# bharatlytics/faceRecognition_InfrenceEngine

Measured on AMD Instinct MI355X. Metric: faces/sec end-to-end @1080p, higher is better.
Workload: dtype f16

## Files before the change

### facerecognition_infrenceengine_amd/_lib.py

```python
import ctypes as C
import struct
import os
import threading

_HERE = os.path.dirname(os.path.abspath(__file__))
LIB_PATH = os.path.join(_HERE, "csrc", "libfrhip.so")

_lock = threading.Lock()
_lib = None
ABI_VERSION = 106


class FrError(RuntimeError):
    pass


class ConvArgs(C.Structure):
    _fields_ = [("x", C.c_void_p), ("w", C.c_void_p), ("y", C.c_void_p),
                ("bias", C.c_void_p), ("slope", C.c_void_p), ("residual", C.c_void_p),
                ("out_f32_partial", C.c_void_p),
                ("B", C.c_int), ("H", C.c_int), ("W", C.c_int), ("Cin", C.c_int), ("Cout", C.c_int),
                ("KH", C.c_int), ("KW", C.c_int), ("stride", C.c_int), ("pad", C.c_int),
                ("Ho", C.c_int), ("Wo", C.c_int), ("bias_mode", C.c_int), ("splitk", C.c_int),
                ("x2", C.c_void_p), ("C2", C.c_int)]


class ConvStep(C.Structure):
    _fields_ = [("kind", C.c_int), ("args", ConvArgs)]


class ConvF8Args(C.Structure):
    _fields_ = [("x8", C.c_void_p), ("w8", C.c_void_p), ("y16", C.c_void_p), ("y8", C.c_void_p),
                ("oscale", C.c_void_p), ("bias", C.c_void_p), ("slope", C.c_void_p), ("residual", C.c_void_p),
                ("B", C.c_int), ("H", C.c_int), ("W", C.c_int), ("Cin", C.c_int), ("Cout", C.c_int),
                ("bias_mode", C.c_int), ("y8_mul", C.c_float), ("y8_sub", C.c_void_p)]


class RolePtr(C.c_void_p):
    role = None


class PnetLevel(C.Structure):
    _fields_ = [("x1", C.c_void_p), ("head", C.c_void_p), ("workspace", C.c_void_p), ("H1", C.c_int), ("W1", C.c_int),
                ("scale", C.c_float), ("boxes", C.c_void_p), ("scores", C.c_void_p), ("regs", C.c_void_p),
                ("counts", C.c_void_p), ("block_counts", C.c_void_p),
                ("x1s", C.c_void_p), ("hs", C.c_int), ("ws", C.c_int), ("f16", C.c_int)]


class FrameRef(C.Structure):
    _fields_ = [("data", C.c_void_p), ("H", C.c_int32), ("W", C.c_int32), ("nh", C.c_int32), ("nw", C.c_int32),
                ("reserved", C.c_int32 * 2)]


class Call(C.Structure):
    _fields_ = [("fn", C.c_int32), ("nargs", C.c_int32), ("a", C.c_uint64 * 22)]


_P, _I, _L, _F, _Z = C.c_void_p, C.c_int, C.c_int64, C.c_float, C.c_size_t
SEQ_FN = {"fr_dconv_mfma_f32": 1, "fr_pnet23_split_f16": 2, "fr_pnet_candidates": 3, "fr_sort_nms": 4, "fr_box_refine": 5,
          "fr_crop_conv1_f32": 6, "fr_stage_select": 7}

SIGNATURES = {
    "fr_version": (_I, []),
    "fr_last_error_string": (C.c_char_p, []),
    "fr_device_count": (_I, []),
    "fr_l2norm_rows_f32": (_I, [_P, _P, _I, _I, _P]),
    "fr_gallery_match_workspace": (_Z, [_I, _L]),
    "fr_gallery_match_f32": (_I, [_P, _P, _I, _L, _I, _L, _P, _P, _P, _Z, _P, _I, _P]),
    "fr_gallery_match_view_f32": (_I, [_P, _P, _P, _I, _L, _I, _P, _P, _P, _Z, _P]),
    "fr_gallery_topk_workspace": (_Z, [_I, _L, _I]),
    "fr_gallery_topk_f32": (_I, [_P, _P, _I, _L, _I, _I, _L, _P, _P, _P, _Z, _P, _I, _P]),
    "fr_gallery_topk_view_f32": (_I, [_P, _P, _P, _I, _L, _I, _I, _P, _P, _P, _Z, _P]),
    "fr_gallery_update_rows_f32": (_I, [_P, _P, _P, _I, _I, _I, _P]),
    "fr_gallery_match_f16_workspace": (_Z, [_I, _L]),
    "fr_gallery_match_f16": (_I, [_P, _P, _P, _I, _L, _I, _L, _P, _P, _P, _Z, _P, _I, _P]),
    "fr_gallery_match_f8_workspace": (_Z, [_I, _L]),
    "fr_gallery_match_f8": (_I, [_P, _P, _P, _I, _L, _I, _L, _P, _P, _P, _Z, _P, _I, _P]),
    "fr_gallery_update_rows_shadow": (_I, [_P, _P, _I, _P, _P, _I, _I, _I, _P]),
    "fr_gallery_match_view_f16_workspace": (_Z, [_I, _L]),
    "fr_gallery_match_view_f16": (_I, [_P, _P, _P, _P, _I, _L, _L, _I, _P, _P, _P, _Z, _P]),
    "fr_gallery_match_view_f8_workspace": (_Z, [_I, _L]),
    "fr_gallery_match_view_f8": (_I, [_P, _P, _P, _P, _I, _L, _L, _I, _P, _P, _P, _Z, _P]),
    "fr_gallery_topk_f16_workspace": (_Z, [_I, _L, _I]),
    "fr_gallery_topk_f16": (_I, [_P, _P, _P, _I, _L, _I, _I, _L, _P, _P, _P, _P, _P, _Z, _P, _I, _P]),
    "fr_gallery_topk_view_f16_workspace": (_Z, [_I, _L, _I]),
    "fr_gallery_topk_view_f16": (_I, [_P, _P, _P, _P, _I, _L, _L, _I, _I, _P, _P, _P, _P, _P, _Z, _P]),
    "fr_gallery_topk_view_masked_f32": (_I, [_P, _P, _P, _I, _L, _I, _I, _P, _P, _P, _Z, _P, _P]),
    "fr_gallery_match_grouped_workspace": (_Z, [_I, _L]),
    "fr_gallery_match_grouped_f32": (_I, [_P, _P, _P, _P, _P, _I, _I, _L, _L, _I, _P, _P, _P, _Z, _P, _I, _P]),
    "fr_gallery_topk_grouped_workspace": (_Z, [_I, _L, _I]),
    "fr_gallery_topk_grouped_f32": (_I, [_P, _P, _P, _P, _P, _I, _I, _L, _L, _I, _I, _P, _P, _P, _Z, _P, _I, _P]),
    "fr_gallery_gmax_update": (_I, [_P, _P, _L, _I, _P, _P]),
    "fr_f32_to_f8": (_I, [_P, _P, _L, _P]),
    "fr_f32_to_f16": (_I, [_P, _P, _L, _P]),
    "fr_match_decide": (_I, [_P, _P, _I, _F, _F, _P, _P]),
    "fr_match_pack_candidates": (_I, [_P, _P, _I, _P, _P]),
    "fr_match_reduce_shards": (_I, [_P, _I, _I, _I, _I, _P, _P, _P]),
    "fr_match_reduce_shards_topk": (_I, [_P, _I, _I, _I, _I, _I, _P, _P, _P]),
    "fr_exchange_pack_queries": (_I, [_P, _I, _I, _I, _P, _P]),
    "fr_exchange_counts": (_I, [_P, _I, _I, _I, _P, _P]),
    "fr_gallery_first_above_f32": (_I, [_P, _P, _I, _L, _I, _F, _I, _L, _P, _P, _P, _Z, _P]),
    "fr_cosine_matrix_f32": (_I, [_P, _P, _I, _I, _I, _P, _P]),
    "fr_mean_rows_f32": (_I, [_P, _I, _I, _P, _P]),
    "fr_unknown_assign_batch_f32": (_I, [_P, _P, _I, _I, _F, _P, _P, _P, _I, _I, _P, _P, _P, _P]),
    "fr_gallery_first_above_blocked_f32": (_I, [_P, _P, _P, _P, _I, _L, _I, _F, _I, _L, _P, _P, _P, _Z, _P]),
    "fr_enrol_batch_workspace": (_Z, [_I, _L]),
    "fr_enrol_batch_f32": (_I, [_P, _P, _I, _P, _P, _I, _P, _I, _I, _I, _P, _P, _L, _F, _F, _P, _P, _P, _P, _P, _P, _P, _P,
                                _Z, _P]),
    "fr_gallery_pairs_workspace": (_Z, [_L, _L]),
    "fr_gallery_pairs_above_f16": (_I, [_P, _P, _L, _I, _F, _I, _L, _I, _P, _P, _P, _P, _Z, _P]),
    "fr_conv_nhwc_f16": (_I, [C.POINTER(ConvArgs), _P]),
    "fr_conv_sequence": (_I, [C.POINTER(ConvStep), _I, _P]),
    "fr_conv_inblock_f16": (_I, [C.POINTER(ConvArgs), _P]),
    "fr_conv_nhwc_f8": (_I, [C.POINTER(ConvF8Args), _P]),
    "fr_quantize_f16_f8": (_I, [_P, _P, _L, _F, _P]),
    "fr_quantize_f16_f8_centred": (_I, [_P, _P, _L, _I, _P, _F, _P]),
    "fr_gptq_round_e4m3": (_I, [_P, _P, _P, _P, _I, _I, _P]),
    "fr_conv_stage14_weight_bytes": (_Z, [_I]),
    "fr_conv_stage14_pack": (_I, [_P, _P, _P]),
    "fr_conv_stage14_f16": (_I, [_P, _P, _P, _P, _I, _I, _P]),
    "fr_conv_walk64_weight_bytes": (_Z, [_I]),
    "fr_conv_walk64_pack": (_I, [_P, _P, _I, _P]),
    "fr_conv_walk64_f16": (_I, [_P, _P, _P, _P, _I, _P, _P, _I, _I, _I, _P]),
    "fr_conv_stage28_weight_bytes": (_Z, [_I]),
    "fr_conv_stage28_pack": (_I, [_P, _P, _P]),
    "fr_conv_stage28_f16": (_I, [_P, _P, _P, _P, _I, _I, _P]),
    "fr_conv_stage14_f8_weight_bytes": (_Z, [_I]),
    "fr_conv_stage14_f8_param_floats": (_Z, []),
    "fr_conv_stage14_f8_pack": (_I, [_P, _P, _P]),
    "fr_conv_stage14_f8": (_I, [_P, _P, _P, _P, _P, _I, _I, _P]),
    "fr_conv_splitk_epilogue": (_I, [_P, _I, _I, _I, _I, _I, _P, _I, _P, _P, _P, _P]),
    "fr_fc_reduce_l2norm": (_I, [_P, _I, _I, _I, _P, _P, _P, _P]),
    "fr_warp_affine_5pt": (_I, [_P, _I, _I, _I, _P, _P, _P, _I, _I, _P, _P, _P, _P]),
    "fr_warp_affine_5pt_slots": (_I, [_P, _I, _I, _I, _P, _P, _I, _I, _P, _P]),
    "fr_warp_affine_5pt_refs": (_I, [_P, _I, _P, _P, _P, _I, _I, _P, _P, _P, _P]),
    "fr_warp_affine_5pt_slots_refs": (_I, [_P, _I, _P, _P, _I, _I, _P, _P]),
    "fr_letterbox_u8": (_I, [_P, _I, _P, _I, _I, _P]),
    "fr_detections_unscale": (_I, [_P, _P, _P, _P, _I, _I, _P]),
    "fr_yuv420_to_bgr_u8": (_I, [_P, _P, _I, _I, _I, _I, _I, _I, _I, _I, _I, _I, _P]),
    "fr_yuv420_to_bgr_refs_u8": (_I, [_P, _P, _I, _I, _I, _I, _I, _I, _I, _I, _P]),
    "fr_frame_activity_u8": (_I, [_P, _I, _I, _I, _P, _I, _P, _P, _P, _I, _P, _P, _P, _I, _I, _I, _P]),
    "fr_frame_activity_refs_u8": (_I, [_P, _I, _P, _I, _P, _P, _P, _I, _P, _P, _P, _I, _I, _I, _P]),
    "fr_hud_draw_u8": (_I, [_P, _I, _I, _I, _P, _I, _P, _P, _I, _P, _I, _P]),
    "fr_hud_draw_refs_u8": (_I, [_P, _I, _P, _I, _P, _P, _I, _P, _I, _P]),
    "fr_track_associate_f32": (_I, [_P, _P, _P, _I, _I, _I, _I, _P, _P, _P, _F, _I, _I, _P, _P, _P, _P]),
    "fr_track_commit_f32": (_I, [_P, _P, _P, _P, _I, _I, _I, _I, _P, _P, _P, _P]),
    "fr_track_resolve_quality_i32": (_I, [_P, _P, _P, _P, _P, _P, _I, _I, _I, _I, _P, _P, _I, _P, _P, _P, _P]),
    "fr_track_fuse_f32": (_I, [_P, _P, _P, _P, _P, _P, _I, _I, _I, _I, _I, _F, _P, _P, _P, _P, _P, _P, _P]),
    "fr_face_quality_f16": (_I, [_P, _P, _P, _I, _I, _P, _P, _P, _F, _I, _I, _I, _I, _I, _F, _F, _F, _P]),
    "fr_pyramid_resize_norm":(_I, [_P, _I, _I, _I, _I, _I, _P, _P]),
    "fr_dconv_f32": (_I, [_P, _P, _P, _P, _P, _I, _I, _I, _I, _I, _I, _I, _I, _I, _P, _P, _I, _P]),
    "fr_dconv_mfma_f32": (_I, [_I, _P, _P, _P, _P, _P, _I, _I, _I, _P, _P, _P, _I, _I, _P, _I, _P, _P]),
    "fr_crop_conv1_f32": (_I, [_I, _P, _I, _I, _I, _P, _P, _I, _P, _P, _P, _P, _P]),
    "fr_crop_conv1_split": (_I, [_I, _P, _I, _I, _I, _P, _P, _I, _P, _P, _P, _P, _I, _P]),
    "fr_crop_conv1_list_f32": (_I, [_I, _P, _I, _I, _I, _P, _I, _P, _P, _I, _P, _P, _P, _P, _P]),
    "fr_ro_conv2_split": (_I, [_I, _P, _P, _P, _P, _P, _I, _P, _I, _P, _P]),
    "fr_ro_gemm_weight_bytes": (_Z, [_I]),
    "fr_ro_gemm_pack": (_I, [_I, _P, _P, _P]),
    "fr_ro_gemm_split": (_I, [_I, _P, _P, _P, _P, _P, _I, _P, _I, _P]),
    "fr_ro_margin_list": (_I, [_P, _I, _P, _I, _I, _F, _F, _P, _P, _I, _P]),
    "fr_ro_scatter_rows": (_I, [_P, _P, _P, _I, _I, _P, _P]),
    "fr_pnet23_workspace_bytes": (_Z, [_I, _I, _I]),
    "fr_pnet23_split_f16": (_I, [_P, _P, _I, _I, _I, _P, _P, _P, _P, _P, _P, _P, _P, _P, _I, _F, _F, _P, _P, _Z, _P]),
    "fr_maxpool_f32": (_I, [_P, _P, _I, _I, _I, _I, _I, _I, _P]),
    "fr_pnet_conv1_band": (_I, [_I, _P, _I, _I, _I, _I, _I, _P, _P, _P, _P, _P, _P, _P, _I, _P]),
    "fr_pnet_band_tiles_count": (_Z, [_I, _I, _I]),
    "fr_pnet_band_tiles": (_I, [_P, _I, _I, _I, _P, _P, _P]),
    "fr_pnet23_coarse_workspace_bytes": (_Z, [_I, _I, _I]),
    "fr_pnet23_coarse_f16": (_I, [_P, _P, _I, _I, _I, _P, _P, _P, _P, _P, _P, _P, _P, _P, _I, _F, _F, _P, _P, _Z, _F, _P, _Z, _P, _P]),
    "fr_pnet_pyramid_p23_coarse": (_I, [C.POINTER(PnetLevel), _I, _I, _P, _P, _P, _P, _P, _P, _P, _P, _I, _F, _F, _F, C.POINTER(_P), _P, _P]),
    "fr_pnet_finish_levels": (_I, [C.POINTER(PnetLevel), _I, _I, _P, _P, _P, _P, _P, _P, _P, _P, _F, _I, _F, _P, _P]),
    "fr_pnet_pyramid_conv1": (_I, [_I, _P, _I, _I, _I, C.POINTER(PnetLevel), _I, _P, _P, _P, _P, _P, _I, _P]),
    "fr_pnet_pyramid_p23": (_I, [C.POINTER(PnetLevel), _I, _I, _P, _P, _P, _P, _P, _P, _P, _P, _I, _F, _F, _P]),
    "fr_pnet_pyramid_band_tiles": (_I, [C.POINTER(PnetLevel), _I, _I, _P, _P, _P]),
    "fr_pnet_candidates": (_I, [_P, _I, _I, _I, _F, _F, _I, _P, _P, _P, _P, _P, _P, _P, _F, _P]),
    "fr_sort_nms": (_I, [_P, _P, _P, _I, _P, _I, _I, _I, _I, _F, _I, _I, _P, _P, _P, _P, _I, _P]),
    "fr_box_refine": (_I, [_P, _P, _I, _P, _I, _I, _I, _P]),
    "fr_crop_resize_norm": (_I, [_P, _I, _I, _I, _P, _P, _I, _I, _P, _P]),
    "fr_stage_select": (_I, [_P, _P, _I, _P, _I, _I, _F, _P, _P, _P, _I, _P, _P, _P]),
    "fr_detect_sequence": (_I, [C.POINTER(Call), _I]),
    "fr_det_conv_weight_halves": (_Z, [_I, _I, _I]),
    "fr_det_conv_f16": (_I, [_P, _P, _P, _P, _P, _I, _I, _I, _I, _I, _I, _I, _I, _I, _I, _I, _I, _I, _I, _I, _P]),
    "fr_det_conv_act_f16": (_I, [_P, _P, _P, _P, _P, _P, _I, _I, _I, _I, _I, _I, _I, _I, _I, _I, _I, _I, _I, _I, _I, _P]),
    "fr_dw_conv_f16": (_I, [_P, _P, _P, _P, _P, _I, _I, _I, _I, _I, _I, _I, _I, _I, _I, _P]),
    "fr_det_input_f16": (_I, [_P, _P, _I, _I, _I, _P]),
    "fr_det_pool_f16": (_I, [_P, _P, _I, _I, _I, _I, _I, _I, _I, _I, _I, _I, _P]),
    "fr_det_upsample_add_f16": (_I, [_P, _P, _P, _I, _I, _I, _I, _I, _P]),
    "fr_scrfd_decode": (_I, [_P, _P, _P, _I, _I, _I, _I, _I, _I, _F, _P, _I, _P, _P, _P, _P, _P]),
}

_NOCHECK = ("fr_version", "fr_device_count")


def _slot(v, t):
    if t is _F:
        return struct.unpack("<I", struct.pack("<f", float(v)))[0]
    if t is _P:
        if v is None:
            return 0
        return int(v.value or 0) if isinstance(v, C.c_void_p) else int(v)
    return int(v) & 0xFFFFFFFFFFFFFFFF


class Lib:

    def __init__(self, cdll):
        self._c = cdll
        self._calls = {}
        self._rec = threading.local()
        for name, (res, args) in SIGNATURES.items():
            fn = getattr(cdll, name)
            fn.restype = res
            fn.argtypes = args
            if res is _I and name not in _NOCHECK:
                self._calls[name] = self._checked(name, fn)
            else:
                self._calls[name] = fn

    def _checked(self, name, fn):
        err = self._c.fr_last_error_string

        fid, types, rec = SEQ_FN.get(name), fn.argtypes, self._rec

        def call(*a):
            rc = fn(*a)
            if rc != 0:
                raise FrError(f"{name} failed ({rc}): {err().decode()}")
            if getattr(rec, "calls", None) is not None:
                rec.invalid = name
            return rc

        def call_rec(*a):
            rc = fn(*a)
            if rc != 0:
                raise FrError(f"{name} failed ({rc}): {err().decode()}")
            calls = getattr(rec, "calls", None)
            if calls is not None:
                calls.append((fid, [_slot(v, t) for v, t in zip(a, types)],
                              [(i, v.role) for i, v in enumerate(a) if isinstance(v, RolePtr)]))
            return rc
        return call_rec if fid is not None else call

    def start_recording(self):
        self._rec.calls, self._rec.invalid = [], None

    def note(self, fid, *slots):
        calls = getattr(self._rec, "calls", None)
        if calls is not None:
            calls.append((fid, [int(v.value or 0) if isinstance(v, C.c_void_p) else int(v) for v in slots], []))

    def stop_recording(self):
        calls, self._rec.calls = getattr(self._rec, "calls", None), None
        self._rec.last_invalid = getattr(self._rec, "invalid", None)
        self._rec.invalid = None
        return None if self._rec.last_invalid else calls

    def recording_invalid(self):
        return getattr(self._rec, "last_invalid", None)

    def __getattr__(self, name):
        try:
            return self.__dict__["_calls"][name]
        except KeyError:
            raise AttributeError(name)


def load():
    global _lib
    with _lock:
        if _lib is None:
            import torch
            if not os.path.exists(LIB_PATH):
                raise FrError(f"{LIB_PATH} not built: run `python -c 'import __graft_entry__ as g; g.build()'` "
                              f"or `make -C {os.path.dirname(LIB_PATH)}`; there is no CPU fallback")
            lib = Lib(C.CDLL(LIB_PATH))
            have = lib.fr_version()
            if have != ABI_VERSION:
                raise FrError(f"{LIB_PATH} implements ABI version {have}, this binding needs {ABI_VERSION}: rebuild it "
                              f"(`make -C {os.path.dirname(LIB_PATH)}`)")
            _lib = lib
        return _lib


def ptr(t, role=None):
    if t is None:
        return None
    if role is None:
        return C.c_void_p(t.data_ptr())
    p = RolePtr(t.data_ptr())
    p.role = role
    return p


def stream_ptr():
    import torch
    return C.c_void_p(torch.cuda.current_stream().cuda_stream)


def require_gpu():
    import torch
    if not torch.cuda.is_available():
        raise FrError("no HIP device visible: this engine has no CPU path")
```

### facerecognition_infrenceengine_amd/csrc/pnet_fused.hip

```cpp
#include "detect_math.h"

#define P23_RH 8
#define P23_RW 32
#define P23_X1W (P23_RW + 4)
#define P23_X1PX ((P23_RH + 4) * P23_X1W)
#define P23_X2W (P23_RW + 2)
#define P23_X2PX ((P23_RH + 2) * P23_X2W)
#define P23_X2T ((P23_X2PX + 15) / 16)
#define P23_NT 512
#define P23_X1PL (448 * 32)
#define P23_X2PL (P23_X2PX * 32)

struct P23Args {
    const float* x1;
    const unsigned char* x1s;
    unsigned x1s_bytes;
    const float* w2; const float* b2; const float* s2;
    const float* w3; const float* b3; const float* s3;
    const float* hw; const float* hb;
    float* head;
    float* dl;
    int all_heads;
    int* list; int* counts; int seg_cap;
    float logit_thr;
    float band_hi;
    int B, H1, W1, H3, W3, tiles_x, tiles_y, ntiles;
    int* clist; int* ccounts;
    float coarse_thr;
    int* visited;
};

template <int NP, int NT>
__device__ __forceinline__ void p23_stage_weights(const P23Args& a, char* wf, float* cst) {
    const int tid = threadIdx.x;
    for (int e = tid; e < 15 * NP * 64; e += NT) {
        const int l2 = e & 63, plane = NP == 2 ? (e >> 6) & 1 : 0, slot = e / (64 * NP);
        const int r = l2 & 15, q = l2 >> 4;
        const bool c3 = slot >= 5;
        const int ct = c3 ? (slot - 5) / 5 : 0, ks = c3 ? (slot - 5) % 5 : slot;
        const float* w = (c3 ? a.w3 : a.w2) + ((size_t)(ct * 16 + r) * 10 + 2 * ks + (q >> 1)) * 16 + 8 * (q & 1);
        half8 o;
#pragma unroll
        for (int j = 0; j < 8; ++j) o[j] = split_f16_plane(w[j], plane);
        *reinterpret_cast<half8*>(wf + (size_t)e * 16) = o;
    }
    for (int e = tid; e < 16; e += NT) { cst[e] = a.b2[e]; cst[16 + e] = a.s2[e] - 1.f; }
    for (int e = tid; e < 32; e += NT) { cst[32 + e] = a.b3[e]; cst[64 + e] = a.s3[e] - 1.f; }
    for (int e = tid; e < 8; e += NT) cst[96 + e] = e < 6 ? a.hb[e] : 0.f;
}

template <bool COARSE>
__device__ __forceinline__ void pnet23_body(const P23Args& a, const int vb, const int vgrid, char* lds) {
#if defined(__HIP_DEVICE_COMPILE__)
    constexpr int NP = COARSE ? 1 : 2;
    char* x1t = lds;
    char* x2t = x1t + NP * P23_X1PL;
    char* wf = x2t + NP * P23_X2PL;
    float* cst = reinterpret_cast<float*>(wf + NP * 15 * 1024);
    int* lcnt = reinterpret_cast<int*>(cst + 104);
    const int tid = threadIdx.x, lane = tid & 63, wave = tid >> 6;
    const int fr = lane & 15, fq = lane >> 4;

    p23_stage_weights<NP, P23_NT>(a, wf, cst);
    if (tid == 0) *lcnt = 0;
    int* const seg = (COARSE ? a.clist : a.list) + (size_t)vb * a.seg_cap;

    int off2[5], off3[5];
#pragma unroll
    for (int ks = 0; ks < 5; ++ks) {
        int t = 2 * ks + (fq >> 1);
        if (t > 8) t = 8;
        off2[ks] = ((t / 3) * P23_X1W + t % 3) * 32 + (fq & 1) * 16;
        off3[ks] = ((t / 3) * P23_X2W + t % 3) * 32 + (fq & 1) * 16;
    }

    __amdgpu_buffer_rsrc_t xrs = buffer_rsrc(a.x1s, a.x1s_bytes);
    constexpr int NPIECE = 14 * NP, NI = (NPIECE + 7) / 8;
    int wy[NI], wx[NI], wc[NI];
#pragma unroll
    for (int i = 0; i < NI; ++i) {
        const int j = wave + 8 * i, pl = j >= 14 ? 1 : 0;
        const int p = (j - 14 * pl) * 32 + (lane >> 1);
        wy[i] = p < P23_X1PX ? p / P23_X1W : 1 << 20; wx[i] = p % P23_X1W;
        wc[i] = pl * 32 + (lane & 1) * 16;
    }
    auto issue_window = [&](int tile) {
        const int per = a.tiles_x * a.tiles_y;
        const int n = tile / per, rem = tile - n * per;
        const int ty0 = (rem / a.tiles_x) * P23_RH, tx0 = (rem % a.tiles_x) * P23_RW;
#pragma unroll
        for (int i = 0; i < NI; ++i) {
            const int j = wave + 8 * i;
            if (j < NPIECE) {
                const int gy = ty0 + wy[i], gx = tx0 + wx[i];
                const unsigned off = (gy < a.H1 && gx < a.W1) ? (unsigned)(((n * a.H1 + gy) * a.W1 + gx) * 64 + wc[i]) : 0x80000000u;
                __builtin_amdgcn_raw_ptr_buffer_load_lds(xrs, (lds_ptr_t)(x1t + (j >= 14 ? P23_X1PL + (j - 14) * 1024 : j * 1024)), 16, off, 0, 0, 0);
            }
        }
    };

    __syncthreads();
    half8 hwh, hwl;
#pragma unroll
    for (int j = 0; j < 8; ++j) {
        const int co = j < 4 ? 4 * fq + j : 16 + 4 * fq + (j - 4);
        const float w = fr < 6 ? a.hw[co * 6 + fr] : 0.f;
        split_f16(w, hwh, hwl, j);
    }
    (void)hwl;
    issue_window(vb);
    for (int tile = vb; tile < a.ntiles; tile += vgrid) {
        const int per = a.tiles_x * a.tiles_y;
        const int n = tile / per, rem = tile - n * per;
        const int ty0 = (rem / a.tiles_x) * P23_RH, tx0 = (rem % a.tiles_x) * P23_RW;
        asm volatile("s_waitcnt vmcnt(0)" ::: "memory");
        __syncthreads();
        {
            const int t0 = wave < 6 ? wave * 3 : 18 + (wave - 6) * 2, nt = wave < 6 ? 3 : 2;
            int pb[3];
            float4v acc[3];
#pragma unroll
            for (int t = 0; t < 3; ++t) {
                int q = (t0 + t) * 16 + fr;
                if (q >= P23_X2PX) q = 0;
                pb[t] = ((q / P23_X2W) * P23_X1W + q % P23_X2W) * 32;
                acc[t] = float4v{0.f, 0.f, 0.f, 0.f};
            }
#pragma unroll
            for (int ks = 0; ks < 5; ++ks) {
                const half8 ahi = *reinterpret_cast<const half8*>(wf + ((ks * NP + 0) * 64 + lane) * 16);
                if constexpr (COARSE) {
#pragma unroll
                    for (int t = 0; t < 3; ++t) {
                        if (t < nt) {
                            const half8 bhi = *reinterpret_cast<const half8*>(x1t + (pb[t] + off2[ks]));
                            acc[t] = __builtin_amdgcn_mfma_f32_16x16x32_f16(ahi, bhi, acc[t], 0, 0, 0);
                        }
                    }
                } else {
                    const half8 alo = *reinterpret_cast<const half8*>(wf + ((ks * 2 + 1) * 64 + lane) * 16);
#pragma unroll
                    for (int t = 0; t < 3; ++t) {
                        if (t < nt) {
                            const char* bp = x1t + (pb[t] + off2[ks]);
                            const half8 bhi = *reinterpret_cast<const half8*>(bp);
                            const half8 blo = *reinterpret_cast<const half8*>(bp + P23_X1PL);
                            acc[t] = __builtin_amdgcn_mfma_f32_16x16x32_f16(alo, bhi, acc[t], 0, 0, 0);
                            acc[t] = __builtin_amdgcn_mfma_f32_16x16x32_f16(ahi, blo, acc[t], 0, 0, 0);
                            acc[t] = __builtin_amdgcn_mfma_f32_16x16x32_f16(ahi, bhi, acc[t], 0, 0, 0);
                        }
                    }
                }
            }
            const float4v bb = *reinterpret_cast<const float4v*>(cst + 4 * fq), ss = *reinterpret_cast<const float4v*>(cst + 16 + 4 * fq);
#pragma unroll
            for (int t = 0; t < 3; ++t) {
                const int q = (t0 + t) * 16 + fr;
                if (t < nt && q < P23_X2PX) {
                    float4v v = acc[t] + bb;
#pragma unroll
                    for (int e = 0; e < 4; ++e) v[e] = __builtin_fmaf(fminf(v[e], 0.f), ss[e], v[e]);
                    char* o = x2t + q * 32 + fq * 8;
                    if constexpr (COARSE) {
                        half4 hi;
#pragma unroll
                        for (int e = 0; e < 4; ++e) hi[e] = (half_t)v[e];
                        *reinterpret_cast<half4*>(o) = hi;
                    } else {
                        half4 hi, lo;
#pragma unroll
                        for (int e = 0; e < 4; ++e) split_f16(v[e], hi, lo, e);
                        *reinterpret_cast<half4*>(o) = hi;
                        *reinterpret_cast<half4*>(o + P23_X2PL) = lo;
                    }
                }
            }
        }
        __syncthreads();
        if (tile + vgrid < a.ntiles) issue_window(tile + vgrid);
        {
            int pb[2];
            float4v acc[2][2];
#pragma unroll
            for (int t = 0; t < 2; ++t) {
                const int q = (wave * 2 + t) * 16 + fr;
                pb[t] = ((q >> 5) * P23_X2W + (q & 31)) * 32;
                acc[t][0] = acc[t][1] = float4v{0.f, 0.f, 0.f, 0.f};
            }
#pragma unroll
            for (int ks = 0; ks < 5; ++ks) {
                if constexpr (COARSE) {
                    half8 ahi[2];
#pragma unroll
                    for (int ct = 0; ct < 2; ++ct) ahi[ct] = *reinterpret_cast<const half8*>(wf + ((5 + ct * 5 + ks) * 64 + lane) * 16);
#pragma unroll
                    for (int t = 0; t < 2; ++t) {
                        const half8 bhi = *reinterpret_cast<const half8*>(x2t + (pb[t] + off3[ks]));
#pragma unroll
                        for (int ct = 0; ct < 2; ++ct) acc[t][ct] = __builtin_amdgcn_mfma_f32_16x16x32_f16(ahi[ct], bhi, acc[t][ct], 0, 0, 0);
                    }
                    continue;
                }
                half8 ahi[2], alo[2];
#pragma unroll
                for (int ct = 0; ct < 2; ++ct) {
                    ahi[ct] = *reinterpret_cast<const half8*>(wf + (((5 + ct * 5 + ks) * 2 + 0) * 64 + lane) * 16);
                    alo[ct] = *reinterpret_cast<const half8*>(wf + (((5 + ct * 5 + ks) * 2 + 1) * 64 + lane) * 16);
                }
#pragma unroll
                for (int t = 0; t < 2; ++t) {
                    const char* bp = x2t + (pb[t] + off3[ks]);
                    const half8 bhi = *reinterpret_cast<const half8*>(bp);
                    const half8 blo = *reinterpret_cast<const half8*>(bp + P23_X2PL);
#pragma unroll
                    for (int ct = 0; ct < 2; ++ct) {
                        acc[t][ct] = __builtin_amdgcn_mfma_f32_16x16x32_f16(alo[ct], bhi, acc[t][ct], 0, 0, 0);
                        acc[t][ct] = __builtin_amdgcn_mfma_f32_16x16x32_f16(ahi[ct], blo, acc[t][ct], 0, 0, 0);
                        acc[t][ct] = __builtin_amdgcn_mfma_f32_16x16x32_f16(ahi[ct], bhi, acc[t][ct], 0, 0, 0);
                    }
                }
            }
            const float4v b30 = *reinterpret_cast<const float4v*>(cst + 32 + 4 * fq), s30 = *reinterpret_cast<const float4v*>(cst + 64 + 4 * fq);
            const float4v b31 = *reinterpret_cast<const float4v*>(cst + 48 + 4 * fq), s31 = *reinterpret_cast<const float4v*>(cst + 80 + 4 * fq);
#pragma unroll
            for (int t = 0; t < 2; ++t) {
                float4v v0 = acc[t][0] + b30, v1 = acc[t][1] + b31;
                half8 bh, bl;
#pragma unroll
                for (int e = 0; e < 4; ++e) {
                    const float x0 = __builtin_fmaf(fminf(v0[e], 0.f), s30[e], v0[e]), x1 = __builtin_fmaf(fminf(v1[e], 0.f), s31[e], v1[e]);
                    const half_t h0 = (half_t)x0, h1 = (half_t)x1;
                    bh[e] = h0; bl[e] = (half_t)(x0 - (float)h0);
                    bh[4 + e] = h1; bl[4 + e] = (half_t)(x1 - (float)h1);
                }
                float4v d = {0.f, 0.f, 0.f, 0.f};
                if constexpr (!COARSE) {
                    d = __builtin_amdgcn_mfma_f32_16x16x32_f16(hwl, bh, d, 0, 0, 0);
                    d = __builtin_amdgcn_mfma_f32_16x16x32_f16(hwh, bl, d, 0, 0, 0);
                }
                d = __builtin_amdgcn_mfma_f32_16x16x32_f16(hwh, bh, d, 0, 0, 0);
                const int q = (wave * 2 + t) * 16 + fr;
                const int gy = ty0 + (q >> 5), gx = tx0 + (q & 31);
                const bool inb = fq < 2 && gy < a.H3 && gx < a.W3;
                const size_t cell = ((size_t)n * a.H3 + gy) * a.W3 + gx;
                const float4v hb4 = *reinterpret_cast<const float4v*>(cst + 96 + 4 * (fq & 1));
                const float o0 = d[0] + hb4[0], o1 = d[1] + hb4[1];
                const float dlv = __shfl(o1 - o0, fr, 64);
                const bool band = a.band_hi > a.logit_thr;
                const bool flag = inb && fq == 0 && (split_nonfinite(dlv) || (COARSE ? dlv >= a.coarse_thr : (dlv >= a.logit_thr && (!band || dlv <= a.band_hi))));
                const unsigned long long fm = __ballot(flag);
                if (fm) {
                    int base = 0;
                    if (lane == (int)__builtin_ctzll(fm)) base = atomicAdd(lcnt, (int)__builtin_popcountll(fm));
                    base = __shfl(base, (int)__builtin_ctzll(fm), 64);
                    if (flag) seg[base + (int)__builtin_popcountll(fm & ((1ull << lane) - 1ull))] = (int)cell;
                }
                if (inb) {
                    if (fq == 0) a.dl[cell] = o1 - o0;
                    if (!COARSE && (a.all_heads || (band && dlv >= a.logit_thr))) {
                        float* o = a.head + cell * 6 + 4 * fq;
                        *reinterpret_cast<float2*>(o) = make_float2(o0, o1);
                        if (fq == 0) *reinterpret_cast<float2*>(o + 2) = make_float2(d[2] + hb4[2], d[3] + hb4[3]);
                    }
                }
            }
        }
    }
    __syncthreads();
    if (tid == 0) (COARSE ? a.ccounts : a.counts)[vb] = *lcnt;
#endif
}

__global__ __launch_bounds__(P23_NT, 4) void pnet23_split_f16(P23Args a) {
    extern __shared__ __attribute__((aligned(16))) char lds[];
    pnet23_body<false>(a, (int)blockIdx.x, (int)gridDim.x, lds);
}
__global__ __launch_bounds__(P23_NT, 4) void pnet23_coarse_f16(P23Args a) {
    extern __shared__ __attribute__((aligned(16))) char lds[];
    pnet23_body<true>(a, (int)blockIdx.x, (int)gridDim.x, lds);
}

#define P23_MAXL 16
struct P23Levels {
    const unsigned char* x1s[P23_MAXL]; float* head[P23_MAXL]; float* dl[P23_MAXL];
    int H1[P23_MAXL], W1[P23_MAXL], seg_cap[P23_MAXL], first[P23_MAXL + 1];
    int nlevels;
};
__global__ __launch_bounds__(P23_NT, 4) void pnet23_split_levels(P23Args a, P23Levels t) {
    extern __shared__ __attribute__((aligned(16))) char lds[];
    int l = 0;
    while (l + 1 < t.nlevels && (int)blockIdx.x >= t.first[l + 1]) ++l;
    a.H1 = t.H1[l]; a.W1 = t.W1[l]; a.H3 = a.H1 - 4; a.W3 = a.W1 - 4;
    a.tiles_x = (a.W3 + P23_RW - 1) / P23_RW; a.tiles_y = (a.H3 + P23_RH - 1) / P23_RH;
    a.ntiles = a.B * a.tiles_x * a.tiles_y;
    a.x1s = t.x1s[l]; a.x1s_bytes = (unsigned)a.B * a.H1 * a.W1 * 64; a.head = t.head[l];
    a.dl = t.dl[l]; a.counts = reinterpret_cast<int*>(a.dl + (size_t)a.B * a.H3 * a.W3); a.list = a.counts + 512;
    a.seg_cap = t.seg_cap[l];
    pnet23_body<false>(a, (int)blockIdx.x - t.first[l], t.first[l + 1] - t.first[l], lds);
}

struct P23Coarse { int* buf[P23_MAXL]; };
__device__ __forceinline__ int p23_find_level(const P23Levels& t, const int g) {
    int l = 0;
    while (l + 1 < t.nlevels && g >= t.first[l + 1]) ++l;
    return l;
}
__device__ __forceinline__ void p23_set_level(P23Args& a, const P23Levels& t, const P23Coarse& c, const int l) {
    a.H1 = t.H1[l]; a.W1 = t.W1[l]; a.H3 = a.H1 - 4; a.W3 = a.W1 - 4;
    a.tiles_x = (a.W3 + P23_RW - 1) / P23_RW; a.tiles_y = (a.H3 + P23_RH - 1) / P23_RH;
    a.ntiles = a.B * a.tiles_x * a.tiles_y;
    a.x1s = t.x1s[l]; a.x1s_bytes = (unsigned)a.B * a.H1 * a.W1 * 64; a.head = t.head[l];
    a.dl = t.dl[l]; a.counts = reinterpret_cast<int*>(a.dl + (size_t)a.B * a.H3 * a.W3); a.list = a.counts + 512;
    a.seg_cap = t.seg_cap[l];
    a.ccounts = c.buf[l]; a.clist = c.buf[l] + 512;
}
__global__ __launch_bounds__(P23_NT, 4) void pnet23_coarse_levels(P23Args a, P23Levels t, P23Coarse c) {
    extern __shared__ __attribute__((aligned(16))) char lds[];
    const int l = p23_find_level(t, (int)blockIdx.x);
    p23_set_level(a, t, c, l);
    pnet23_body<true>(a, (int)blockIdx.x - t.first[l], t.first[l + 1] - t.first[l], lds);
}

#define P23R_NT 256
#define P23R_SLOT 1616
#define P23R_LO 800
#define P23R_LDS ((size_t)30 * 1024 + 108 * 4 + (P23R_NT / 64) * 16 * P23R_SLOT)
__global__ __launch_bounds__(P23R_NT, 1) void pnet23_reeval_levels(P23Args a, P23Levels t, P23Coarse c) {
#if defined(__HIP_DEVICE_COMPILE__)
    extern __shared__ __attribute__((aligned(16))) char lds[];
    char* wf = lds;
    float* cst = reinterpret_cast<float*>(wf + 30 * 1024);
    const int tid = threadIdx.x, lane = tid & 63, wave = tid >> 6;
    const int fr = lane & 15, fq = lane >> 4;
    char* const win = reinterpret_cast<char*>(cst + 108) + wave * (16 * P23R_SLOT);
    p23_stage_weights<2, P23R_NT>(a, wf, cst);
    half8 hwh, hwl;
#pragma unroll
    for (int j = 0; j < 8; ++j) {
        const int co = j < 4 ? 4 * fq + j : 16 + 4 * fq + (j - 4);
        const float w = fr < 6 ? a.hw[co * 6 + fr] : 0.f;
        split_f16(w, hwh, hwl, j);
    }
    __syncthreads();
    const float4v bb = *reinterpret_cast<const float4v*>(cst + 4 * fq), ss = *reinterpret_cast<const float4v*>(cst + 16 + 4 * fq);
    const float4v b30 = *reinterpret_cast<const float4v*>(cst + 32 + 4 * fq), s30 = *reinterpret_cast<const float4v*>(cst + 64 + 4 * fq);
    const float4v b31 = *reinterpret_cast<const float4v*>(cst + 48 + 4 * fq), s31 = *reinterpret_cast<const float4v*>(cst + 80 + 4 * fq);
    const float4v hb4 = *reinterpret_cast<const float4v*>(cst + 96 + 4 * (fq & 1));
    const bool band = a.band_hi > a.logit_thr;
    char* const xc = win + fr * P23R_SLOT + (fq & 1) * 16;
    int pj[25], psrc[25], pdst[25];
    const int nseg = t.first[t.nlevels];
    for (int g = (int)blockIdx.x * (P23R_NT / 64) + wave; g < nseg; g += (int)gridDim.x * (P23R_NT / 64)) {
        const int l = p23_find_level(t, g);
        p23_set_level(a, t, c, l);
        const int vb = g - t.first[l];
        const int n_list = a.ccounts[vb];
        const int* const lst = a.clist + (size_t)vb * a.seg_cap;
        int* const seg = a.list + (size_t)vb * a.seg_cap;
        const int hw3 = a.H3 * a.W3;
        int nflag = 0;
        if (a.visited && lane == 0 && n_list) atomicAdd(a.visited, n_list);
#pragma unroll
        for (int it = 0; it < 25; ++it) {
            const int idx = it * 64 + lane, j = idx / 100, rem = idx - j * 100, px = rem >> 2, ch = rem & 3;
            pj[it] = j;
            psrc[it] = ((px / 5) * a.W1 + px % 5) * 64 + ch * 16;
            pdst[it] = j * P23R_SLOT + (ch >> 1) * P23R_LO + px * 32 + (ch & 1) * 16;
        }
        auto corner_of = [&](int i0) {
            const int cell = lst[min(i0 + fr, n_list - 1)];
            const int n = cell / hw3, rem = cell - n * hw3, y = rem / a.W3, x = rem - y * a.W3;
            return ((n * a.H1 + y) * a.W1 + x) * 64;
        };
        float4v pf[25];
        if (n_list > 0) {
            const int corner = corner_of(0);
#pragma unroll
            for (int it = 0; it < 25; ++it)
                pf[it] = *reinterpret_cast<const float4v*>(a.x1s + (size_t)(unsigned)(__shfl(corner, pj[it], 64) + psrc[it]));
        }
        for (int i0 = 0; i0 < n_list; i0 += 16) {
            const int cell = lst[min(i0 + fr, n_list - 1)];
#pragma unroll
            for (int it = 0; it < 25; ++it) *reinterpret_cast<float4v*>(win + pdst[it]) = pf[it];
            __builtin_amdgcn_wave_barrier();
            if (i0 + 16 < n_list) {
                const int corner = corner_of(i0 + 16);
#pragma unroll
                for (int it = 0; it < 25; ++it)
                    pf[it] = *reinterpret_cast<const float4v*>(a.x1s + (size_t)(unsigned)(__shfl(corner, pj[it], 64) + psrc[it]));
            }
            float4v acc2[9];
#pragma unroll
            for (int p = 0; p < 9; ++p) acc2[p] = float4v{0.f, 0.f, 0.f, 0.f};
#pragma unroll
            for (int ks = 0; ks < 5; ++ks) {
                int tp = 2 * ks + (fq >> 1);
                if (tp > 8) tp = 8;
                const half8 ahi = *reinterpret_cast<const half8*>(wf + ((ks * 2 + 0) * 64 + lane) * 16);
                const half8 alo = *reinterpret_cast<const half8*>(wf + ((ks * 2 + 1) * 64 + lane) * 16);
#pragma unroll
                for (int p = 0; p < 9; ++p) {
                    const char* bp = xc + ((p / 3 + tp / 3) * 5 + (p % 3 + tp % 3)) * 32;
                    const half8 bhi = *reinterpret_cast<const half8*>(bp);
                    const half8 blo = *reinterpret_cast<const half8*>(bp + P23R_LO);
                    acc2[p] = __builtin_amdgcn_mfma_f32_16x16x32_f16(alo, bhi, acc2[p], 0, 0, 0);
                    acc2[p] = __builtin_amdgcn_mfma_f32_16x16x32_f16(ahi, blo, acc2[p], 0, 0, 0);
                    acc2[p] = __builtin_amdgcn_mfma_f32_16x16x32_f16(ahi, bhi, acc2[p], 0, 0, 0);
                }
            }
            __builtin_amdgcn_wave_barrier();
#pragma unroll
            for (int p = 0; p < 9; ++p) {
                float4v v = acc2[p] + bb;
#pragma unroll
                for (int e = 0; e < 4; ++e) v[e] = __builtin_fmaf(fminf(v[e], 0.f), ss[e], v[e]);
                half4 hi, lo;
#pragma unroll
                for (int e = 0; e < 4; ++e) split_f16(v[e], hi, lo, e);
                char* o = win + fr * P23R_SLOT + p * 32 + fq * 8;
                *reinterpret_cast<half4*>(o) = hi;
                *reinterpret_cast<half4*>(o + P23R_LO) = lo;
            }
            __builtin_amdgcn_wave_barrier();
            float4v acc3[2] = {float4v{0.f, 0.f, 0.f, 0.f}, float4v{0.f, 0.f, 0.f, 0.f}};
#pragma unroll
            for (int ks = 0; ks < 5; ++ks) {
                int tp = 2 * ks + (fq >> 1);
                if (tp > 8) tp = 8;
                const half8 bhi = *reinterpret_cast<const half8*>(xc + tp * 32);
                const half8 blo = *reinterpret_cast<const half8*>(xc + tp * 32 + P23R_LO);
#pragma unroll
                for (int ct = 0; ct < 2; ++ct) {
                    const half8 ahi = *reinterpret_cast<const half8*>(wf + (((5 + ct * 5 + ks) * 2 + 0) * 64 + lane) * 16);
                    const half8 alo = *reinterpret_cast<const half8*>(wf + (((5 + ct * 5 + ks) * 2 + 1) * 64 + lane) * 16);
                    acc3[ct] = __builtin_amdgcn_mfma_f32_16x16x32_f16(alo, bhi, acc3[ct], 0, 0, 0);
                    acc3[ct] = __builtin_amdgcn_mfma_f32_16x16x32_f16(ahi, blo, acc3[ct], 0, 0, 0);
                    acc3[ct] = __builtin_amdgcn_mfma_f32_16x16x32_f16(ahi, bhi, acc3[ct], 0, 0, 0);
                }
            }
            __builtin_amdgcn_wave_barrier();
            const float4v v0 = acc3[0] + b30, v1 = acc3[1] + b31;
            half8 bh, bl;
#pragma unroll
            for (int e = 0; e < 4; ++e) {
                const float x0 = __builtin_fmaf(fminf(v0[e], 0.f), s30[e], v0[e]), x1 = __builtin_fmaf(fminf(v1[e], 0.f), s31[e], v1[e]);
                const half_t h0 = (half_t)x0, h1 = (half_t)x1;
                bh[e] = h0; bl[e] = (half_t)(x0 - (float)h0);
                bh[4 + e] = h1; bl[4 + e] = (half_t)(x1 - (float)h1);
            }
            float4v d = {0.f, 0.f, 0.f, 0.f};
            d = __builtin_amdgcn_mfma_f32_16x16x32_f16(hwl, bh, d, 0, 0, 0);
            d = __builtin_amdgcn_mfma_f32_16x16x32_f16(hwh, bl, d, 0, 0, 0);
            d = __builtin_amdgcn_mfma_f32_16x16x32_f16(hwh, bh, d, 0, 0, 0);
            const bool inb = fq < 2 && i0 + fr < n_list;
            const float o0 = d[0] + hb4[0], o1 = d[1] + hb4[1];
            const float dlv = __shfl(o1 - o0, fr, 64);
            const bool flag = inb && fq == 0 && (split_nonfinite(dlv) || (dlv >= a.logit_thr && (!band || dlv <= a.band_hi)));
            const unsigned long long fm = __ballot(flag);
            if (flag) seg[nflag + (int)__builtin_popcountll(fm & ((1ull << lane) - 1ull))] = cell;
            nflag += (int)__builtin_popcountll(fm);
            if (inb) {
                if (fq == 0) a.dl[cell] = o1 - o0;
                if (band && dlv >= a.logit_thr) {
                    float* o = a.head + (size_t)cell * 6 + 4 * fq;
                    *reinterpret_cast<float2*>(o) = make_float2(o0, o1);
                    if (fq == 0) *reinterpret_cast<float2*>(o + 2) = make_float2(d[2] + hb4[2], d[3] + hb4[3]);
                }
            }
        }
        if (lane == 0) a.counts[vb] = nflag;
    }
#endif
}

#define PREF_WS 304
struct PRefArgs {
    const float* x1; const float* w2; const float* b2; const float* s2; const float* w3; const float* b3; const float* s3;
    const float* hw; const float* hb; float* head;
    const int* list; const int* counts; int seg_cap;
    int B, H1, W1, H3, W3;
    int* counter;
};

__device__ __forceinline__ void pnet_refine_body(const PRefArgs& a, const int block, float (*wins)[16 * PREF_WS], int (*cbase)[16]) {
#if defined(__HIP_DEVICE_COMPILE__)
    const int tid = threadIdx.x, lane = tid & 63, wave = tid >> 6;
    const int li = lane & 15, kq = lane >> 4;
    float* win = wins[wave];
    if (a.counts[block] <= wave * 16) return;
    float wa2[27], wa3[2][36], hwa[8];
#pragma unroll
    for (int s = 0; s < 27; ++s) wa2[s] = a.w2[(li * 10 + s / 3) * 16 + 4 * (s % 3) + kq];
#pragma unroll
    for (int i = 0; i < 2; ++i)
#pragma unroll
        for (int s = 0; s < 36; ++s) wa3[i][s] = a.w3[((16 * i + li) * 10 + s / 4) * 16 + 4 * (s % 4) + kq];
#pragma unroll
    for (int i = 0; i < 2; ++i)
#pragma unroll
        for (int e = 0; e < 4; ++e) hwa[i * 4 + e] = li < 6 ? a.hw[(16 * i + 4 * kq + e) * 6 + li] : 0.f;
    const float4v b2 = *reinterpret_cast<const float4v*>(a.b2 + 4 * kq), s2 = *reinterpret_cast<const float4v*>(a.s2 + 4 * kq);
    float4v b3[2], s3[2], hb4;
#pragma unroll
    for (int i = 0; i < 2; ++i) {
        b3[i] = *reinterpret_cast<const float4v*>(a.b3 + 16 * i + 4 * kq);
        s3[i] = *reinterpret_cast<const float4v*>(a.s3 + 16 * i + 4 * kq);
    }
#pragma unroll
    for (int r = 0; r < 4; ++r) hb4[r] = kq * 4 + r < 6 ? a.hb[kq * 4 + r] : 0.f;

    const int hw3 = a.H3 * a.W3;
    {
        const int* lst = a.list + (size_t)block * a.seg_cap;
        const int n_list = a.counts[block];
        if (a.counter && tid == 0 && n_list) atomicAdd(a.counter, n_list);
        for (int i0 = wave * 16; i0 < n_list; i0 += 64) {
            {
                const int c = lst[min(i0 + li, n_list - 1)];
                const int n = c / hw3, r = c - n * hw3, y = r / a.W3, x = r - y * a.W3;
                if (kq == 0) cbase[wave][li] = ((n * a.H1 + y) * a.W1 + x) * 12;
            }
            __builtin_amdgcn_wave_barrier();
            int l_ = lane;
            asm volatile("" : "+v"(l_));
            float4v pf[19];
#pragma unroll
            for (int it = 0; it < 19; ++it) {
                const int idx = min(it * 64 + l_, 1199);
                const int j = idx / 75, rem = idx - j * 75, row = rem / 15, c4 = rem - row * 15;
                pf[it] = *reinterpret_cast<const float4v*>(a.x1 + (size_t)(unsigned)cbase[wave][j] + (row * a.W1 * 12 + c4 * 4));
            }
#pragma unroll
            for (int it = 0; it < 19; ++it) {
                const int idx = it * 64 + l_;
                const int j = idx / 75, rem = idx - j * 75, row = rem / 15, c4 = rem - row * 15;
                if (it < 18 || l_ < 48) *reinterpret_cast<float4v*>(win + j * PREF_WS + row * 60 + c4 * 4) = pf[it];
            }
            __builtin_amdgcn_wave_barrier();
            const float* xb = win + li * PREF_WS + kq;
            float4v acc2[9];
#pragma unroll
            for (int p = 0; p < 9; ++p) acc2[p] = float4v{0.f, 0.f, 0.f, 0.f};
#pragma unroll
            for (int s = 0; s < 27; ++s) {
                const int tap = s / 3, c4 = s - tap * 3, ty = tap / 3, tx = tap - ty * 3;
#pragma unroll
                for (int p = 0; p < 9; ++p) {
                    const int py = p / 3, px = p - py * 3;
                    acc2[p] = __builtin_amdgcn_mfma_f32_16x16x4f32(wa2[s], xb[((py + ty) * 5 + px + tx) * 12 + 4 * c4], acc2[p], 0, 0, 0);
                }
            }
            __builtin_amdgcn_wave_barrier();
#pragma unroll
            for (int p = 0; p < 9; ++p) {
                float4v v = acc2[p] + b2;
#pragma unroll
                for (int e = 0; e < 4; ++e) v[e] = v[e] > 0.f ? v[e] : v[e] * s2[e];
                *reinterpret_cast<float4v*>(win + li * PREF_WS + p * 16 + 4 * kq) = v;
            }
            __builtin_amdgcn_wave_barrier();
            float4v acc3[2] = {float4v{0.f, 0.f, 0.f, 0.f}, float4v{0.f, 0.f, 0.f, 0.f}};
#pragma unroll
            for (int s = 0; s < 36; ++s) {
                const float bv = xb[(s / 4) * 16 + 4 * (s % 4)];
#pragma unroll
                for (int i = 0; i < 2; ++i) acc3[i] = __builtin_amdgcn_mfma_f32_16x16x4f32(wa3[i][s], bv, acc3[i], 0, 0, 0);
            }
            float4v hd = hb4;
#pragma unroll
            for (int i = 0; i < 2; ++i) {
                float4v v = acc3[i] + b3[i];
#pragma unroll
                for (int e = 0; e < 4; ++e) v[e] = v[e] > 0.f ? v[e] : v[e] * s3[i][e];
#pragma unroll
                for (int e = 0; e < 4; ++e) hd = __builtin_amdgcn_mfma_f32_16x16x4f32(hwa[i * 4 + e], v[e], hd, 0, 0, 0);
            }
            if (i0 + li < n_list && kq < 2) {
                float* o = a.head + (size_t)lst[i0 + li] * 6 + 4 * kq;
                *reinterpret_cast<float2*>(o) = make_float2(hd[0], hd[1]);
                if (kq == 0) *reinterpret_cast<float2*>(o + 2) = make_float2(hd[2], hd[3]);
            }
            __builtin_amdgcn_wave_barrier();
        }
    }
#endif
}

__global__ __launch_bounds__(256, 2) void pnet_refine_mfma(PRefArgs a) {
    __shared__ __attribute__((aligned(16))) float wins[4][16 * PREF_WS];
    __shared__ int cbase[4][16];
    pnet_refine_body(a, blockIdx.x, wins, cbase);
}

#define PREF_MAXL 16
struct PRefLevels {
    const float* x1[PREF_MAXL]; float* head[PREF_MAXL]; const int* list[PREF_MAXL]; const int* counts[PREF_MAXL];
    int seg_cap[PREF_MAXL], H1[PREF_MAXL], W1[PREF_MAXL], first[PREF_MAXL + 1];
    int nlevels;
};
__global__ __launch_bounds__(256, 2) void pnet_refine_levels(PRefArgs a, PRefLevels t) {
    __shared__ __attribute__((aligned(16))) float wins[4][16 * PREF_WS];
    __shared__ int cbase[4][16];
    int l = 0;
    while (l + 1 < t.nlevels && (int)blockIdx.x >= t.first[l + 1]) ++l;
    a.x1 = t.x1[l]; a.head = t.head[l]; a.list = t.list[l]; a.counts = t.counts[l]; a.seg_cap = t.seg_cap[l];
    a.H1 = t.H1[l]; a.W1 = t.W1[l]; a.H3 = t.H1[l] - 4; a.W3 = t.W1[l] - 4;
    pnet_refine_body(a, (int)blockIdx.x - t.first[l], wins, cbase);
}

static void p23_layout(int B, int H1, int W1, long long& ncell, long long& ntiles, int& grid, int& seg_cap) {
    const int H3 = H1 - 4, W3 = W1 - 4;
    ncell = (long long)B * H3 * W3;
    ntiles = (long long)B * ((W3 + P23_RW - 1) / P23_RW) * ((H3 + P23_RH - 1) / P23_RH);
    grid = (int)(ntiles < 512 ? ntiles : 512);
    seg_cap = (int)((ntiles + grid - 1) / (grid > 0 ? grid : 1)) * (P23_RH * P23_RW);
}
extern "C" size_t fr_pnet23_workspace_bytes(int B, int H1, int W1) {
    if (B <= 0 || H1 < 5 || W1 < 5) return 0;
    long long ncell, ntiles; int grid, seg_cap;
    p23_layout(B, H1, W1, ncell, ntiles, grid, seg_cap);
    return (size_t)ncell * 4 + 512 * 4 + (size_t)grid * seg_cap * 4;
}

extern "C" size_t fr_pnet23_coarse_workspace_bytes(int B, int H1, int W1) {
    if (B <= 0 || H1 < 5 || W1 < 5) return 0;
    long long ncell, ntiles; int grid, seg_cap;
    p23_layout(B, H1, W1, ncell, ntiles, grid, seg_cap);
    return 512 * 4 + (size_t)grid * seg_cap * 4;
}

static unsigned p23_reeval_grid(long long segments) {
    const long long blocks = (segments + P23R_NT / 64 - 1) / (P23R_NT / 64);
    return (unsigned)(blocks < 256 ? blocks : 256);
}

constexpr size_t P23_LDS = (size_t)2 * P23_X1PL + (size_t)2 * P23_X2PL + 30 * 1024 + 108 * 4;
constexpr size_t P23C_LDS = (size_t)P23_X1PL + (size_t)P23_X2PL + 15 * 1024 + 108 * 4;

static int p23_level(const char* who, const float* x1, const void* x1s, int B, int H1, int W1, const float* w2, const float* b2,
                     const float* s2, const float* w3, const float* b3, const float* s3, const float* hw,
                     const float* hb, float* head, int all_heads, float refine_logit_thr, float refine_band_hi,
                     int32_t* refined_count, void* workspace, size_t workspace_bytes, float coarse_margin, void* coarse,
                     size_t coarse_bytes, int32_t* visited_count, fr_stream_t stream);

extern "C" int fr_pnet23_split_f16(const float* x1, const void* x1s, int B, int H1, int W1, const float* w2, const float* b2,
                                   const float* s2, const float* w3, const float* b3, const float* s3, const float* hw,
                                   const float* hb, float* head, int all_heads, float refine_logit_thr, float refine_band_hi,
                                   int32_t* refined_count, void* workspace, size_t workspace_bytes, fr_stream_t stream) {
    return p23_level("fr_pnet23_split_f16", x1, x1s, B, H1, W1, w2, b2, s2, w3, b3, s3, hw, hb, head, all_heads, refine_logit_thr,
                     refine_band_hi, refined_count, workspace, workspace_bytes, 0.f, nullptr, 0, nullptr, stream);
}

extern "C" int fr_pnet23_coarse_f16(const float* x1, const void* x1s, int B, int H1, int W1, const float* w2, const float* b2,
                                    const float* s2, const float* w3, const float* b3, const float* s3, const float* hw,
                                    const float* hb, float* head, int all_heads, float refine_logit_thr, float refine_band_hi,
                                    int32_t* refined_count, void* workspace, size_t workspace_bytes, float coarse_margin,
                                    void* coarse, size_t coarse_bytes, int32_t* visited_count, fr_stream_t stream) {
    FR_REQUIRE(!(all_heads & 1), "fr_pnet23_coarse_f16: all_heads & 1 (the approximate heads of every cell) needs fr_pnet23_split_f16");
    FR_REQUIRE(coarse && coarse_margin >= 0.f, "fr_pnet23_coarse_f16: needs a coarse buffer and a margin >= 0");
    return p23_level("fr_pnet23_coarse_f16", x1, x1s, B, H1, W1, w2, b2, s2, w3, b3, s3, hw, hb, head, all_heads, refine_logit_thr,
                     refine_band_hi, refined_count, workspace, workspace_bytes, coarse_margin, coarse, coarse_bytes, visited_count, stream);
}

static int p23_level(const char* who, const float* x1, const void* x1s, int B, int H1, int W1, const float* w2, const float* b2,
                     const float* s2, const float* w3, const float* b3, const float* s3, const float* hw,
                     const float* hb, float* head, int all_heads, float refine_logit_thr, float refine_band_hi,
                     int32_t* refined_count, void* workspace, size_t workspace_bytes, float coarse_margin, void* coarse,
                     size_t coarse_bytes, int32_t* visited_count, fr_stream_t stream) {
    FR_REQUIRE(x1 && x1s && w2 && b2 && s2 && w3 && b3 && s3 && hw && hb && head, "%s: null pointer", who);
    FR_REQUIRE((int64_t)B * H1 * W1 * 64 < (1ll << 31), "%s: the split conv1 map must stay below 2 GiB (got %lld bytes)", who, (long long)B * H1 * W1 * 64);
    FR_REQUIRE(B > 0 && H1 >= 5 && W1 >= 5, "%s: the conv1 map must be at least 5x5 (got %dx%d)", who, H1, W1);
    P23Args a;
    a.x1 = x1; a.x1s = (const unsigned char*)x1s; a.x1s_bytes = (unsigned)((int64_t)B * H1 * W1 * 64); a.w2 = w2; a.b2 = b2; a.s2 = s2; a.w3 = w3; a.b3 = b3; a.s3 = s3; a.hw = hw; a.hb = hb; a.head = head; a.all_heads = all_heads & 1;
    a.B = B; a.H1 = H1; a.W1 = W1; a.H3 = H1 - 4; a.W3 = W1 - 4;
    a.tiles_x = (a.W3 + P23_RW - 1) / P23_RW; a.tiles_y = (a.H3 + P23_RH - 1) / P23_RH;
    long long ncell, nt; int grid, seg_cap;
    p23_layout(B, H1, W1, ncell, nt, grid, seg_cap);
    FR_REQUIRE(nt < (1ll << 31) && ncell < (1ll << 31), "%s: too many tiles", who);
    const size_t need = fr_pnet23_workspace_bytes(B, H1, W1);
    FR_REQUIRE(workspace && workspace_bytes >= need, "%s: workspace needs %zu bytes (fr_pnet23_workspace_bytes)", who, need);
    a.dl = reinterpret_cast<float*>(workspace);
    a.counts = reinterpret_cast<int*>(a.dl + ncell);
    a.list = a.counts + 512;
    a.seg_cap = seg_cap;
    a.logit_thr = refine_logit_thr;
    a.band_hi = refine_band_hi;
    a.ntiles = (int)nt;
    a.clist = a.ccounts = a.visited = nullptr; a.coarse_thr = 0.f;
    hipStream_t s = fr_stream(stream);
    if (coarse) {
        const size_t cneed = fr_pnet23_coarse_workspace_bytes(B, H1, W1);
        FR_REQUIRE(coarse_bytes >= cneed, "%s: the coarse buffer needs %zu bytes (fr_pnet23_coarse_workspace_bytes)", who, cneed);
        a.ccounts = reinterpret_cast<int*>(coarse); a.clist = a.ccounts + 512;
        a.coarse_thr = refine_logit_thr - coarse_margin; a.visited = visited_count;
        static FrDevLatch latch0, latch1;
        if (!fr_raise_lds(reinterpret_cast<const void*>(pnet23_coarse_f16), P23C_LDS, latch0) ||
            !fr_raise_lds(reinterpret_cast<const void*>(pnet23_reeval_levels), P23R_LDS, latch1)) { fr_set_error("fr_pnet23_coarse_f16: cannot raise dynamic LDS"); return FR_E_LAUNCH; }
        pnet23_coarse_f16<<<grid, P23_NT, P23C_LDS, s>>>(a);
        FR_CHECK_LAUNCH("pnet23_coarse_f16");
        P23Levels t{};
        P23Coarse c{};
        t.nlevels = 1; t.x1s[0] = a.x1s; t.head[0] = head; t.dl[0] = a.dl; t.H1[0] = H1; t.W1[0] = W1; t.seg_cap[0] = seg_cap;
        t.first[0] = 0; t.first[1] = grid; c.buf[0] = a.ccounts;
        pnet23_reeval_levels<<<p23_reeval_grid(grid), P23R_NT, P23R_LDS, s>>>(a, t, c);
        FR_CHECK_LAUNCH("pnet23_reeval_levels");
    } else {
        static FrDevLatch latch;
        if (!fr_raise_lds(reinterpret_cast<const void*>(pnet23_split_f16), P23_LDS, latch)) { fr_set_error("fr_pnet23_split_f16: cannot raise dynamic LDS"); return FR_E_LAUNCH; }
        pnet23_split_f16<<<grid, P23_NT, P23_LDS, s>>>(a);
        FR_CHECK_LAUNCH("pnet23_split_f16");
    }
    if (all_heads & 2) return FR_OK;
    PRefArgs r;
    r.x1 = x1; r.w2 = w2; r.b2 = b2; r.s2 = s2; r.w3 = w3; r.b3 = b3; r.s3 = s3; r.hw = hw; r.hb = hb; r.head = head;
    r.list = a.list; r.counts = a.counts; r.seg_cap = seg_cap;
    r.B = B; r.H1 = H1; r.W1 = W1; r.H3 = a.H3; r.W3 = a.W3; r.counter = refined_count;
    pnet_refine_mfma<<<grid, 256, 0, s>>>(r);
    FR_CHECK_LAUNCH("pnet_refine_mfma");
    return FR_OK;
}

int fr_pnet_candidates_levels_launch(const fr_pnet_level* lv, int nlevels, int nframes, float thr, int cap, float dl_min, hipStream_t s);

extern "C" int fr_pnet_finish_levels(const fr_pnet_level* levels, int nlevels, int nframes, const float* w2, const float* b2,
                                     const float* s2, const float* w3, const float* b3, const float* s3, const float* hw,
                                     const float* hb, float thr, int cap, float dl_min, int32_t* refined_count, fr_stream_t stream) {
    FR_REQUIRE(levels && nlevels > 0 && nlevels <= PREF_MAXL && nframes > 0 && cap > 0, "fr_pnet_finish_levels: 1 .. %d levels", PREF_MAXL);
    FR_REQUIRE(w2 && b2 && s2 && w3 && b3 && s3 && hw && hb, "fr_pnet_finish_levels: null pointer");
    PRefLevels t;
    t.nlevels = nlevels;
    int total = 0;
    for (int l = 0; l < nlevels; ++l) {
        const fr_pnet_level& L = levels[l];
        FR_REQUIRE(L.x1 && L.head && L.workspace && L.boxes && L.scores && L.regs && L.counts && L.block_counts && L.H1 >= 5 && L.W1 >= 5 && L.scale > 0.f,
                   "fr_pnet_finish_levels: level %d: bad entry", l);
        long long ncell, nt; int grid, seg_cap;
        p23_layout(nframes, L.H1, L.W1, ncell, nt, grid, seg_cap);
        float* dl = reinterpret_cast<float*>(L.workspace);
        const int* counts = reinterpret_cast<const int*>(dl + ncell);
        t.x1[l] = L.x1; t.head[l] = L.head; t.counts[l] = counts; t.list[l] = counts + 512;
        t.seg_cap[l] = seg_cap; t.H1[l] = L.H1; t.W1[l] = L.W1;
        t.first[l] = total;
        total += grid;
    }
    t.first[nlevels] = total;
    PRefArgs r;
    r.x1 = nullptr; r.w2 = w2; r.b2 = b2; r.s2 = s2; r.w3 = w3; r.b3 = b3; r.s3 = s3; r.hw = hw; r.hb = hb; r.head = nullptr;
    r.list = nullptr; r.counts = nullptr; r.seg_cap = 0; r.B = nframes; r.H1 = r.W1 = r.H3 = r.W3 = 0; r.counter = refined_count;
    hipStream_t s = fr_stream(stream);
    pnet_refine_levels<<<total, 256, 0, s>>>(r, t);
    FR_CHECK_LAUNCH("pnet_refine_levels");
    return fr_pnet_candidates_levels_launch(levels, nlevels, nframes, thr, cap, dl_min, s);
}

__global__ __launch_bounds__(256) void pnet_band_tiles_kernel(const int* __restrict__ list, const int* __restrict__ counts, int seg_cap,
                                                             int H3, int W3, int regions_x, int regions_y, int32_t* __restrict__ tbuf,
                                                             int32_t* __restrict__ tiles) {
    const int n_list = counts[blockIdx.x];
    const int* lst = list + (size_t)blockIdx.x * seg_cap;
    const int hw3 = H3 * W3;
    for (int i = threadIdx.x; i < n_list; i += 256) {
        const int c = lst[i];
        const int n = c / hw3, r = c - n * hw3, y = r / W3, x = r - y * W3;
        const int ry0 = (2 * y) >> 4, ry1 = min((2 * y + 9) >> 4, regions_y - 1);
        const int rx0 = (2 * x) >> 6, rx1 = min((2 * x + 9) >> 6, regions_x - 1);
        for (int ry = ry0; ry <= ry1; ++ry)
            for (int rx = rx0; rx <= rx1; ++rx) {
                const int t = (n * regions_y + ry) * regions_x + rx;
                const unsigned bit = 1u << (t & 31);
                const unsigned old = atomicOr(reinterpret_cast<unsigned*>(tbuf) + 1 + (t >> 5), bit);
                if (!(old & bit)) tiles[atomicAdd(tbuf, 1)] = t;
            }
    }
}

extern "C" size_t fr_pnet_band_tiles_count(int B, int H1, int W1) {
    if (B <= 0 || H1 < 5 || W1 < 5) return 0;
    return (size_t)B * ((H1 + 7) / 8) * ((W1 + 31) / 32);
}

extern "C" int fr_pnet_band_tiles(const void* workspace, int B, int H1, int W1, int32_t* tbuf, int32_t* tiles, fr_stream_t stream) {
    FR_REQUIRE(workspace && tbuf && tiles && B > 0 && H1 >= 5 && W1 >= 5, "fr_pnet_band_tiles: bad argument");
    long long ncell, nt; int grid, seg_cap;
    p23_layout(B, H1, W1, ncell, nt, grid, seg_cap);
    const float* dl = reinterpret_cast<const float*>(workspace);
    const int* counts = reinterpret_cast<const int*>(dl + ncell);
    const int regions_y = (H1 + 7) / 8, regions_x = (W1 + 31) / 32;
    const size_t ntile = (size_t)B * regions_y * regions_x;
    hipStream_t s = fr_stream(stream);
    if (hipMemsetAsync(tbuf, 0, (1 + (ntile + 31) / 32) * sizeof(int32_t), s) != hipSuccess) { fr_set_error("fr_pnet_band_tiles: memset failed"); return FR_E_LAUNCH; }
    pnet_band_tiles_kernel<<<grid, 256, 0, s>>>(counts + 512, counts, seg_cap, H1 - 4, W1 - 4, regions_x, regions_y, tbuf, tiles);
    FR_CHECK_LAUNCH("pnet_band_tiles_kernel");
    return FR_OK;
}

static int p23_pyramid(const char* who, const fr_pnet_level* levels, int nlevels, int nframes, const float* w2, const float* b2,
                       const float* s2, const float* w3, const float* b3, const float* s3, const float* hw,
                       const float* hb, int all_heads, float refine_logit_thr, float refine_band_hi, float coarse_margin,
                       void* const* coarse, int32_t* visited_count, fr_stream_t stream);

extern "C" int fr_pnet_pyramid_p23(const fr_pnet_level* levels, int nlevels, int nframes, const float* w2, const float* b2,
                                   const float* s2, const float* w3, const float* b3, const float* s3, const float* hw,
                                   const float* hb, int all_heads, float refine_logit_thr, float refine_band_hi, fr_stream_t stream) {
    return p23_pyramid("fr_pnet_pyramid_p23", levels, nlevels, nframes, w2, b2, s2, w3, b3, s3, hw, hb, all_heads, refine_logit_thr,
                       refine_band_hi, 0.f, nullptr, nullptr, stream);
}

extern "C" int fr_pnet_pyramid_p23_coarse(const fr_pnet_level* levels, int nlevels, int nframes, const float* w2, const float* b2,
                                          const float* s2, const float* w3, const float* b3, const float* s3, const float* hw,
                                          const float* hb, int all_heads, float refine_logit_thr, float refine_band_hi,
                                          float coarse_margin, void* const* coarse, int32_t* visited_count, fr_stream_t stream) {
    FR_REQUIRE(!(all_heads & 1), "fr_pnet_pyramid_p23_coarse: all_heads & 1 (the approximate heads of every cell) needs fr_pnet_pyramid_p23");
    FR_REQUIRE(coarse && coarse_margin >= 0.f, "fr_pnet_pyramid_p23_coarse: needs the coarse buffers and a margin >= 0");
    return p23_pyramid("fr_pnet_pyramid_p23_coarse", levels, nlevels, nframes, w2, b2, s2, w3, b3, s3, hw, hb, all_heads, refine_logit_thr,
                       refine_band_hi, coarse_margin, coarse, visited_count, stream);
}

static int p23_pyramid(const char* who, const fr_pnet_level* levels, int nlevels, int nframes, const float* w2, const float* b2,
                       const float* s2, const float* w3, const float* b3, const float* s3, const float* hw,
                       const float* hb, int all_heads, float refine_logit_thr, float refine_band_hi, float coarse_margin,
                       void* const* coarse, int32_t* visited_count, fr_stream_t stream) {
    FR_REQUIRE(levels && nlevels > 0 && nlevels <= P23_MAXL && nframes > 0, "%s: 1 .. %d levels", who, P23_MAXL);
    FR_REQUIRE(w2 && b2 && s2 && w3 && b3 && s3 && hw && hb, "%s: null pointer", who);
    P23Levels t;
    P23Coarse c{};
    t.nlevels = nlevels;
    long long total = 0;
    for (int l = 0; l < nlevels; ++l) {
        const fr_pnet_level& L = levels[l];
        if (coarse) {
            FR_REQUIRE(coarse[l], "%s: level %d: no coarse buffer", who, l);
            c.buf[l] = reinterpret_cast<int*>(coarse[l]);
        }
        FR_REQUIRE(L.x1s && L.head && L.workspace && L.H1 >= 5 && L.W1 >= 5, "%s: level %d: bad entry", who, l);
        FR_REQUIRE((int64_t)nframes * L.H1 * L.W1 * 64 < (1ll << 31), "%s: level %d: the split conv1 map must stay below 2 GiB", who, l);
        long long ncell, nt; int grid, seg_cap;
        p23_layout(nframes, L.H1, L.W1, ncell, nt, grid, seg_cap);
        t.x1s[l] = reinterpret_cast<const unsigned char*>(L.x1s); t.head[l] = L.head; t.dl[l] = reinterpret_cast<float*>(L.workspace);
        t.H1[l] = L.H1; t.W1[l] = L.W1; t.seg_cap[l] = seg_cap;
        t.first[l] = (int)total;
        total += grid;
    }
    t.first[nlevels] = (int)total;
    P23Args a{};
    a.w2 = w2; a.b2 = b2; a.s2 = s2; a.w3 = w3; a.b3 = b3; a.s3 = s3; a.hw = hw; a.hb = hb; a.all_heads = all_heads & 1;
    a.logit_thr = refine_logit_thr; a.band_hi = refine_band_hi; a.B = nframes;
    if (coarse) {
        a.coarse_thr = refine_logit_thr - coarse_margin; a.visited = visited_count;
        static FrDevLatch latch0, latch1;
        if (!fr_raise_lds(reinterpret_cast<const void*>(pnet23_coarse_levels), P23C_LDS, latch0) ||
            !fr_raise_lds(reinterpret_cast<const void*>(pnet23_reeval_levels), P23R_LDS, latch1)) { fr_set_error("fr_pnet_pyramid_p23_coarse: cannot raise dynamic LDS"); return FR_E_LAUNCH; }
        pnet23_coarse_levels<<<(unsigned)total, P23_NT, P23C_LDS, fr_stream(stream)>>>(a, t, c);
        FR_CHECK_LAUNCH("pnet23_coarse_levels");
        pnet23_reeval_levels<<<p23_reeval_grid(total), P23R_NT, P23R_LDS, fr_stream(stream)>>>(a, t, c);
        FR_CHECK_LAUNCH("pnet23_reeval_levels");
        return FR_OK;
    }
    static FrDevLatch latch;
    if (!fr_raise_lds(reinterpret_cast<const void*>(pnet23_split_levels), P23_LDS, latch)) { fr_set_error("fr_pnet_pyramid_p23: cannot raise dynamic LDS"); return FR_E_LAUNCH; }
    pnet23_split_levels<<<(unsigned)total, P23_NT, P23_LDS, fr_stream(stream)>>>(a, t);
    FR_CHECK_LAUNCH("pnet23_split_levels");
    return FR_OK;
}

struct PBandLevels {
    const int* counts[PREF_MAXL];
    int seg_cap[PREF_MAXL], H1[PREF_MAXL], W1[PREF_MAXL], word0[PREF_MAXL], level[PREF_MAXL], first[PREF_MAXL + 1];
    int nlevels;
};
__global__ __launch_bounds__(256) void pnet_band_tiles_levels(PBandLevels t, int32_t* __restrict__ tbuf, int32_t* __restrict__ tiles, int cap) {
    int l = 0;
    while (l + 1 < t.nlevels && (int)blockIdx.x >= t.first[l + 1]) ++l;
    const int b = (int)blockIdx.x - t.first[l];
    const int n_list = t.counts[l][b];
    const int* lst = t.counts[l] + 512 + (size_t)b * t.seg_cap[l];
    const int H3 = t.H1[l] - 4, W3 = t.W1[l] - 4, hw3 = H3 * W3;
    const int regions_y = (t.H1[l] + 7) / 8, regions_x = (t.W1[l] + 31) / 32;
    unsigned* bitmap = reinterpret_cast<unsigned*>(tbuf) + 1 + t.word0[l];
    for (int i = threadIdx.x; i < n_list; i += 256) {
        const int c = lst[i];
        const int n = c / hw3, r = c - n * hw3, y = r / W3, x = r - y * W3;
        const int ry0 = (2 * y) >> 4, ry1 = min((2 * y + 9) >> 4, regions_y - 1);
        const int rx0 = (2 * x) >> 6, rx1 = min((2 * x + 9) >> 6, regions_x - 1);
        for (int ry = ry0; ry <= ry1; ++ry)
            for (int rx = rx0; rx <= rx1; ++rx) {
                const int tl = (n * regions_y + ry) * regions_x + rx;
                const unsigned bit = 1u << (tl & 31);
                const unsigned old = atomicOr(bitmap + (tl >> 5), bit);
                if (!(old & bit)) {
                    const int at = atomicAdd(tbuf, 1);
                    if (at < cap) tiles[at] = (t.level[l] << 27) | tl;
                }
            }
    }
}

extern "C" int fr_pnet_pyramid_band_tiles(const fr_pnet_level* levels, int nlevels, int nframes, int32_t* tbuf, int32_t* tiles,
                                          fr_stream_t stream) {
    FR_REQUIRE(levels && nlevels > 0 && nlevels <= PREF_MAXL && nframes > 0 && tbuf && tiles, "fr_pnet_pyramid_band_tiles: bad argument");
    PBandLevels t;
    t.nlevels = 0;
    long long blocks = 0, words = 0, cap = 0;
    for (int l = 0; l < nlevels; ++l) {
        const fr_pnet_level& L = levels[l];
        if (!L.f16) continue;
        FR_REQUIRE(L.workspace && L.H1 >= 5 && L.W1 >= 5, "fr_pnet_pyramid_band_tiles: level %d: bad entry", l);
        long long ncell, nt; int grid, seg_cap;
        p23_layout(nframes, L.H1, L.W1, ncell, nt, grid, seg_cap);
        const long long ntile = (long long)fr_pnet_band_tiles_count(nframes, L.H1, L.W1);
        FR_REQUIRE(ntile < (1ll << 27), "fr_pnet_pyramid_band_tiles: level %d: too many tiles", l);
        const int k = t.nlevels++;
        t.counts[k] = reinterpret_cast<const int*>(reinterpret_cast<const float*>(L.workspace) + ncell);
        t.seg_cap[k] = seg_cap; t.H1[k] = L.H1; t.W1[k] = L.W1; t.word0[k] = (int)words; t.level[k] = l;
        t.first[k] = (int)blocks;
        blocks += grid; words += (ntile + 31) / 32; cap += ntile;
    }
    FR_REQUIRE(t.nlevels > 0 && cap < (1ll << 31), "fr_pnet_pyramid_band_tiles: no level in the f16 form");
    t.first[t.nlevels] = (int)blocks;
    hipStream_t s = fr_stream(stream);
    if (hipMemsetAsync(tbuf, 0, (size_t)(1 + words) * sizeof(int32_t), s) != hipSuccess) { fr_set_error("fr_pnet_pyramid_band_tiles: memset failed"); return FR_E_LAUNCH; }
    pnet_band_tiles_levels<<<(unsigned)blocks, 256, 0, s>>>(t, tbuf, tiles, (int)cap);
    FR_CHECK_LAUNCH("pnet_band_tiles_levels");
    return FR_OK;
}
```

### facerecognition_infrenceengine_amd/mtcnn.py

```python
import contextlib
import ctypes
import functools
import logging
import math
import threading
from types import SimpleNamespace
from typing import NamedTuple

import torch

from . import _lib


def pyramid_scales(h, w, minsize=20, factor=0.709):
    m = 12.0 / minsize
    minl = min(h, w) * m
    scales, k = [], 0
    while minl >= 12:
        scales.append(m * factor ** k)
        minl *= factor
        k += 1
    return scales


def _pool_out(n, k, s):
    o = -(-(n - k) // s) + 1
    if (o - 1) * s >= n:
        o -= 1
    return o


MFMA_LAYERS = {0: (3, 12, 3, 3, 1), 1: (12, 16, 3, 3, 1), 2: (16, 32, 3, 3, 2),
               10: (4, 28, 3, 3, 2), 11: (28, 48, 3, 3, 3), 12: (48, 64, 2, 2, 4), 13: (64, 128, 3, 3, 4),
               14: (128, 6, 1, 1, 1),
               20: (4, 32, 3, 3, 1), 21: (32, 64, 3, 3, 2), 22: (64, 64, 3, 3, 4), 23: (64, 128, 2, 2, 4),
               24: (128, 256, 3, 3, 4), 25: (256, 16, 1, 1, 1)}


class _MConv:

    def __init__(self, layer, w, b, slope, device, head=None):
        cin, cout, kh, kw, ntb = MFMA_LAYERS[layer]
        rcout, rcin = w.shape[0], w.shape[1]
        assert tuple(w.shape[2:]) == (kh, kw) and rcout <= cout and rcin <= cin, (layer, tuple(w.shape))
        wfull = torch.zeros((cout, cin, kh, kw), dtype=torch.float32)
        wfull[:rcout, :rcin] = w
        w = wfull
        bfull = torch.zeros(cout); bfull[:rcout] = b; b = bfull
        if slope is not None:
            sfull = torch.zeros(cout); sfull[:rcout] = slope; slope = sfull
        self.layer, self.cin, self.cout, self.kh, self.kw = layer, cin, cout, kh, kw
        cinp = -(-cin // 4) * 4
        cp = ntb * 16 + (16 if ntb % 2 == 0 else 0)
        gsz = ntb * 16
        ngroups = -(-cout // gsz)
        wp = torch.zeros((ngroups, kh * kw, cinp, cp), dtype=torch.float32)
        wt = w.permute(2, 3, 1, 0).reshape(kh * kw, cin, cout)
        for g in range(ngroups):
            n = min(gsz, cout - g * gsz)
            wp[g, :, :cin, :n] = wt[:, :, g * gsz:g * gsz + n]
        self.w = wp.contiguous().to(device)
        bp = torch.zeros(ngroups * gsz); bp[:cout] = b
        self.b = bp.to(device)
        self.slope = None
        if slope is not None:
            sp = torch.zeros(ngroups * gsz); sp[:cout] = slope
            self.slope = sp.to(device)
        self.head_w = self.head_b = None
        self.nhead = 0
        if head is not None:
            self.head_w = head[0].t().contiguous().to(torch.float32).to(device)
            self.head_b = head[1].to(torch.float32).contiguous().to(device)
            self.nhead = head[0].shape[0]
        self.pool = {0: 2, 10: 3, 11: 3, 20: 3, 21: 3, 22: 2}.get(layer, 0)

    def out_hw(self, h, w):
        hc, wc = h - self.kh + 1, w - self.kw + 1
        return (_pool_out(hc, self.pool, 2), _pool_out(wc, self.pool, 2)) if self.pool else (hc, wc)


_CHAINS = {"pnet": (("conv1", ("conv2",)), ("conv2", ("conv3",)), ("conv3", ("conv4_1", "conv4_2"))),
           "rnet": (("conv1", ("conv2",)), ("conv2", ("conv3",)), ("conv3", ("dense4",)), ("dense4", ("dense5_1", "dense5_2"))),
           "onet": (("conv1", ("conv2",)), ("conv2", ("conv3",)), ("conv3", ("conv4",)), ("conv4", ("dense5",)),
                    ("dense5", ("dense6_1", "dense6_2", "dense6_3")))}


def canonical_scale(state, net, dead_zone=2):
    st = dict(state)
    for name, readers in _CHAINS[net]:
        w = st[name + ".weight"]
        rms = float(w.double().pow(2).mean().sqrt())
        if rms == 0.0:
            continue
        e = math.log2(math.sqrt(2.0 / w[0].numel()) / rms)
        k = int(round(e)) if abs(e) > dead_zone else 0
        if k:
            st[name + ".weight"] = w * 2.0 ** k
            st[name + ".bias"] = st[name + ".bias"] * 2.0 ** k
            for n in readers:
                st[n + ".weight"] = st[n + ".weight"] * 2.0 ** -k
    return st


def _dense_as_conv(w, k, c):
    o = w.shape[0]
    return w.reshape(o, k, k, c).permute(0, 3, 2, 1).contiguous()


class DetectSettings:
    SINGLE_FRAME_LEVEL_STREAMS = 4
    one_stream = False
    level_streams = 2
    phase_marks = None
    solo_max_frames = 7
    pnet_band = True
    split_pconv1 = True
    split_pconv1_min_px = 10000
    pyramid_launch = True
    refined_cells = None
    use_sequence = True
    fused_crop = True
    split_ro = True
    coarse_p23 = True
    coarse_margin = 0.05
    visited_cells = None

    def __init__(self, minsize=20, factor=0.709, fused_pnet=True, batch_min_pixels=None):
        self.minsize, self.factor = minsize, factor
        self.fused_pnet = bool(fused_pnet)
        self.batch_min_pixels = 22_000_000 if batch_min_pixels is None else int(batch_min_pixels)
        self.single_frame_level_streams = self.SINGLE_FRAME_LEVEL_STREAMS


class DetectPlan(NamedTuple):
    N: int
    scales: tuple
    geo: tuple
    batch: bool
    few: bool
    band: bool
    fused: tuple
    f16: tuple
    pyramid: bool
    solo: bool
    nside: int
    cache: bool
    recorder: bool
    split: bool
    coarse: float
    chunks: tuple


def _is_batch(cfg, N, H, W):
    return N * H * W >= cfg.batch_min_pixels


def _level_geo(H, W, scale):
    hs, ws = int(math.ceil(H * scale)), int(math.ceil(W * scale))
    return hs, ws, _pool_out(hs - 2, 2, 2), _pool_out(ws - 2, 2, 2)


def _frames32(h, w):
    return (2 ** 31 - 1) // (h * w * 64)


def _f16_conv1(cfg, band, h, w):
    return bool(band and cfg.split_pconv1 and h * w >= cfg.split_pconv1_min_px)


def detect_plan(N, H, W, cfg, trace=False, level_streams=None, out=False, capturing=False):
    return _plan(N, H, W, tuple([getattr(cfg, k) for k in _PLAN_READS]), cfg.phase_marks is None and cfg.refined_cells is None,
                 trace, level_streams, out, capturing)


_PLAN_READS = ("minsize", "factor", "fused_pnet", "batch_min_pixels", "solo_max_frames", "pnet_band", "split_pconv1", "split_pconv1_min_px",
               "pyramid_launch", "one_stream", "level_streams", "single_frame_level_streams", "split_ro", "fused_crop", "use_sequence",
               "coarse_p23", "coarse_margin")


@functools.lru_cache(maxsize=256)
def _plan(N, H, W, settings, recordable, trace, level_streams, out, capturing):
    cfg = SimpleNamespace(**dict(zip(_PLAN_READS, settings)))
    scales = tuple(pyramid_scales(H, W, cfg.minsize, cfg.factor))
    geo = tuple(_level_geo(H, W, s) for s in scales)
    batch = _is_batch(cfg, N, H, W)
    few = N <= cfg.solo_max_frames and not batch
    fusable = bool(cfg.fused_pnet) and not trace
    chunks, per = (), N
    if fusable and not out and N > 1 and geo and 1 <= _frames32(*geo[0][2:]) < N:
        per = -(-N // -(-N // _frames32(*geo[0][2:])))
        chunks = tuple((n0, min(N, n0 + per)) for n0 in range(0, N, per))
    band = bool(cfg.pnet_band and batch and not trace)
    fused = tuple(bool(cfg.fused_pnet) and per <= _frames32(h, w) for _, _, h, w in geo)
    f16 = tuple(fu and _f16_conv1(cfg, band, h, w) for fu, (_, _, h, w) in zip(fused, geo))
    pyramid = bool(cfg.pyramid_launch and batch and fusable and all(fused))
    nside = max(1, min(2, level_streams if level_streams is not None else cfg.level_streams))
    own = few and level_streams is None
    if own and capturing and cfg.single_frame_level_streams > 0:
        nside = min(cfg.single_frame_level_streams, max(1, len(scales) - 1))
    eager = bool(trace or cfg.one_stream or (own and not capturing))
    cache = bool(eager and few and not trace and not out and not capturing)
    recorder = bool(cache and recordable and cfg.use_sequence and cfg.fused_pnet and cfg.fused_crop and not cfg.one_stream)
    split = bool(cfg.split_ro and cfg.fused_crop and batch and not trace)
    coarse = float(cfg.coarse_margin) if cfg.coarse_p23 and band else 0.0
    return DetectPlan(N, scales, geo, batch, few, band, fused, f16, pyramid, eager or pyramid, nside, cache, recorder, split, coarse, chunks)


_RO = (SimpleNamespace(name="rnet", cap_in="cap_p", cap_out="cap_r", crop=24, map1=(11, 28), map2=(4, 48), w1="_rc1", w2="_rc2",
                       layers=("r1", "r2", "r3", "r4", "r5"), nhead=6, naux=4, refine=1),
       SimpleNamespace(name="onet", cap_in="cap_r", cap_out="cap_o", crop=48, map1=(23, 32), map2=(10, 64), w1="_oc1", w2="_oc2",
                       layers=("o1", "o2", "o3", "o4", "o5", "o6"), nhead=16, naux=14, refine=2))


class MTCNNHIP(DetectSettings):
    def __init__(self, pstate, rstate, ostate, device="cuda:0", minsize=20, factor=0.709,
                 thresholds=(0.6, 0.7, 0.7), cap_scale=2048, keep_scale=256, cap_p=512, cap_r=64, cap_o=16,
                 fused_pnet=True, batch_min_pixels=None, canonical=True):
        _lib.require_gpu()
        DetectSettings.__init__(self, minsize, factor, fused_pnet, batch_min_pixels)
        self.lib = _lib.load()
        self.device = torch.device(device)
        self.thresholds = tuple(float(t) for t in thresholds)
        self.cap_scale, self.keep_scale, self.cap_p, self.cap_r, self.cap_o = cap_scale, keep_scale, cap_p, cap_r, cap_o
        assert cap_scale <= 4096 and cap_p <= 1024 and cap_r <= 1024 and cap_o <= 1024
        self._sides = {}
        self._tls = threading.local()
        self._unfused_logged = False
        d = self.device
        p, r, o = ({k: v.detach().float().cpu() for k, v in s.items()} for s in (pstate, rstate, ostate))
        if canonical:
            p, r, o = (canonical_scale(s, n) for s, n in ((p, "pnet"), (r, "rnet"), (o, "onet")))
        self.p1 = _MConv(0, p["conv1.weight"], p["conv1.bias"], p["prelu1.weight"], d)
        self.p2 = _MConv(1, p["conv2.weight"], p["conv2.bias"], p["prelu2.weight"], d)
        hw = torch.cat([p["conv4_1.weight"].reshape(2, 32), p["conv4_2.weight"].reshape(4, 32)])
        hb = torch.cat([p["conv4_1.bias"], p["conv4_2.bias"]])
        self.p3 = _MConv(2, p["conv3.weight"], p["conv3.bias"], p["prelu3.weight"], d, head=(hw, hb))
        w2p = torch.zeros((16, 10, 16)); w2p[:, :9, :10] = p["conv2.weight"].permute(0, 2, 3, 1).reshape(16, 9, 10)
        w3p = torch.zeros((32, 10, 16)); w3p[:, :9, :16] = p["conv3.weight"].permute(0, 2, 3, 1).reshape(32, 9, 16)
        self._p23 = tuple(t.to(torch.float32).contiguous().to(d) for t in (
            w2p, p["conv2.bias"], p["prelu2.weight"], w3p, p["conv3.bias"], p["prelu3.weight"], hw.t().contiguous(), hb))
        self.refine_margin = 2e-3
        self.level_tensors = None
        self.p23_all_heads = False
        self._rc1 = tuple(t.to(torch.float32).contiguous().to(d) for t in (
            r["conv1.weight"].permute(2, 3, 1, 0).reshape(27, 28), r["conv1.bias"], r["prelu1.weight"]))
        self._oc1 = tuple(t.to(torch.float32).contiguous().to(d) for t in (
            o["conv1.weight"].permute(2, 3, 1, 0).reshape(27, 32), o["conv1.bias"], o["prelu1.weight"]))
        self.split_conv1 = True
        self.ro_margin = 1e-3
        self.ro_list_cap = (1024, 256)
        def c2w(w):
            o, c = w.shape[0], w.shape[1]
            wp = torch.zeros((o, 9, 32))
            wp[:, :, :c] = w.permute(0, 2, 3, 1).reshape(o, 9, c)
            return wp
        self._rc2 = tuple(t.to(torch.float32).contiguous().to(d) for t in (c2w(r["conv2.weight"]), r["conv2.bias"], r["prelu2.weight"]))
        self._oc2 = tuple(t.to(torch.float32).contiguous().to(d) for t in (c2w(o["conv2.weight"]), o["conv2.bias"], o["prelu2.weight"]))
        self.r1 = _MConv(10, r["conv1.weight"], r["conv1.bias"], r["prelu1.weight"], d)
        self.r2 = _MConv(11, r["conv2.weight"], r["conv2.bias"], r["prelu2.weight"], d)
        self.r3 = _MConv(12, r["conv3.weight"], r["conv3.bias"], r["prelu3.weight"], d)
        self.r4 = _MConv(13, _dense_as_conv(r["dense4.weight"], 3, 64), r["dense4.bias"], r["prelu4.weight"], d)
        self.r5 = _MConv(14, torch.cat([r["dense5_1.weight"], r["dense5_2.weight"]]).reshape(6, 128, 1, 1),
                         torch.cat([r["dense5_1.bias"], r["dense5_2.bias"]]), None, d)
        self.o1 = _MConv(20, o["conv1.weight"], o["conv1.bias"], o["prelu1.weight"], d)
        self.o2 = _MConv(21, o["conv2.weight"], o["conv2.bias"], o["prelu2.weight"], d)
        self.o3 = _MConv(22, o["conv3.weight"], o["conv3.bias"], o["prelu3.weight"], d)
        self.o4 = _MConv(23, o["conv4.weight"], o["conv4.bias"], o["prelu4.weight"], d)
        self.o5 = _MConv(24, _dense_as_conv(o["dense5.weight"], 3, 128), o["dense5.bias"], o["prelu5.weight"], d)
        self._gemm = {}
        for lid, wconv, b, sl in ((12, r["conv3.weight"], r["conv3.bias"], r["prelu3.weight"]),
                                  (13, _dense_as_conv(r["dense4.weight"], 3, 64), r["dense4.bias"], r["prelu4.weight"]),
                                  (22, o["conv3.weight"], o["conv3.bias"], o["prelu3.weight"]),
                                  (23, o["conv4.weight"], o["conv4.bias"], o["prelu4.weight"]),
                                  (24, _dense_as_conv(o["dense5.weight"], 3, 128), o["dense5.bias"], o["prelu5.weight"])):
            wk = wconv.permute(0, 2, 3, 1).reshape(wconv.shape[0], -1).to(torch.float32).contiguous().to(d)
            packed = torch.empty(self.lib.fr_ro_gemm_weight_bytes(lid), dtype=torch.uint8, device=d)
            with torch.cuda.device(d):
                self.lib.fr_ro_gemm_pack(lid, _lib.ptr(wk), _lib.ptr(packed), _lib.stream_ptr())
                torch.cuda.synchronize(d)
            self._gemm[lid] = (packed, b.to(torch.float32).contiguous().to(d), sl.to(torch.float32).contiguous().to(d))
        self.o6 = _MConv(25, torch.cat([o["dense6_1.weight"], o["dense6_2.weight"], o["dense6_3.weight"]]).reshape(16, 256, 1, 1),
                         torch.cat([o["dense6_1.bias"], o["dense6_2.bias"], o["dense6_3.bias"]]), None, d)

    def set_exact(self, on=True):
        self.pnet_band = self.split_ro = not on
        return self

    @property
    def _dl(self):
        return getattr(self._tls, "dl", (None, 0.0))

    @property
    def _s(self):
        return self._tls.s

    @_s.setter
    def _s(self, v):
        self._tls.s = v

    def _new(self, shape, dtype):
        c = getattr(self._tls, "cache", None)
        if c is None:
            return torch.empty(shape, dtype=dtype, device=self.device)
        lst, i = c
        c[1] = i + 1
        if i < len(lst) and lst[i].shape == tuple(shape) and lst[i].dtype == dtype:
            return lst[i]
        t = torch.empty(shape, dtype=dtype, device=self.device)
        self._tls.cache_grew = True
        if i < len(lst):
            lst[i] = t
        else:
            lst.append(t)
        return t

    def _f32(self, *shape):
        return self._new(shape, torch.float32)

    def _i32(self, *shape):
        return self._new(shape, torch.int32)

    def _fptr(self, frames):
        return _lib.ptr(frames, role="frame")

    def _dconv(self, x, c, B, H, W, frames=None, counts=None, cap=0, y_split=None, y=None):
        ho, wo = c.out_hw(H, W)
        if y is None:
            y = self._f32(B, ho, wo, c.nhead if c.nhead else c.cout)
        fh, fw = (frames.shape[1], frames.shape[2]) if frames is not None else (0, 0)
        self.lib.fr_dconv_mfma_f32(c.layer, _lib.ptr(x), _lib.ptr(c.w), _lib.ptr(c.b), _lib.ptr(c.slope), _lib.ptr(y),
                                   B, H, W, _lib.ptr(c.head_w), _lib.ptr(c.head_b), self._fptr(frames), fh, fw,
                                   _lib.ptr(counts), cap, _lib.ptr(y_split), self._s)
        return y, ho, wo

    def _gemm_split(self, lid, x, B, shape, counts, cap):
        w, b, sl = self._gemm[lid]
        y = self._f32(B, *shape)
        self.lib.fr_ro_gemm_split(lid, _lib.ptr(x), _lib.ptr(w), _lib.ptr(b), _lib.ptr(sl), _lib.ptr(y), B, _lib.ptr(counts), cap, self._s)
        return y

    def _nms(self, boxes, scores, aux, naux, counts, L, nseg, seg_cap, seg_major, thr, mode, keep, out=None, results=False):
        if out is None:
            bo, so, co = self._f32(L, keep, 4), self._f32(L, keep), self._i32(L)
            ao = self._f32(L, keep, max(naux, 1))
        else:
            bo, so, ao, co = out
        po = [_lib.ptr(t, role="out%d" % i if results else None) for i, t in enumerate((bo, so, ao, co))]
        self.lib.fr_sort_nms(_lib.ptr(boxes), _lib.ptr(scores), _lib.ptr(aux), naux, _lib.ptr(counts), L, nseg, seg_cap,
                             seg_major, thr, mode, keep, *po, keep, self._s)
        return bo, so, ao, co

    def _band_logits(self, band=True):
        lt = math.log(self.thresholds[0] / (1.0 - self.thresholds[0]))
        return lt - self.refine_margin, lt + self.refine_margin if band else float("-inf")

    def _coarse(self, margin):
        return 0.0 if self.p23_all_heads else margin

    def _level_buffers(self, N, scale, geo, band, f16, cand, coarse=0.0):
        hs, ws, h, w = geo
        path = getattr(self._tls, "path", None)
        if path is not None:
            path["fused_levels"] += 1
            path["band_levels"] += int(band)
            path["coarse_levels"] += int(coarse > 0.0)
            if f16:
                path["pconv1_mfma_levels"].append((h, w))
        xs = self._new((N, h, w, 64), torch.uint8)
        x = self._f32(N, h, w, 12)
        head = self._f32(N, h - 4, w - 4, 6)
        wsp = self._new((self.lib.fr_pnet23_workspace_bytes(N, h, w) // 4,), torch.float32)
        bc = self._i32(N * (-(-(h - 4) * (w - 4) // 256)))
        cws = self._i32(self.lib.fr_pnet23_coarse_workspace_bytes(N, h, w) // 4) if coarse > 0.0 else None
        entry = None
        if cand is not None:
            entry = _lib.PnetLevel(x.data_ptr(), head.data_ptr(), wsp.data_ptr(), h, w, float(scale), *[t.data_ptr() for t in cand],
                                   bc.data_ptr(), xs.data_ptr(), hs, ws, int(f16))
        return dict(h=h, w=w, f16=f16, x=x, xs=xs, head=head, wsp=wsp, bc=bc, cws=cws), entry

    def _level(self, frames, scale, geo, fused, band, f16, trace, cand, coarse=0.0):
        N, H, W, _ = frames.shape
        hs, ws, h, w = geo
        lib, p1 = self.lib, self.p1
        if not fused:
            if self.fused_pnet and not self._unfused_logged:
                self._unfused_logged = True
                logging.getLogger(__name__).warning("MTCNNHIP: a %d x %d pyramid level of %d frame(s) exceeds the fused P-Net's 32-bit map "
                                                    "offsets; it runs layer by layer (f32)", hs, ws, N)
            if getattr(self._tls, "path", None) is not None:
                self._tls.path["unfused_levels"] += 1
            x, h, w = self._dconv(None, p1, N, hs, ws, frames=frames)
            x, h, w = self._dconv(x, self.p2, N, h, w)
            head, h, w = self._dconv(x, self.p3, N, h, w)
            return head, h, w, self._i32(N * (-(-h * w // 256))), None, 0.0, None
        lo, hi = self._band_logits(band)
        coarse = self._coarse(coarse)
        t, entry = self._level_buffers(N, scale, geo, band, f16, cand[3:] if f16 else None, coarse)
        x, xs, head, wsp, cws = t["x"], t["xs"], t["head"], t["wsp"], t["cws"]
        p1w, p23 = (_lib.ptr(p1.w), _lib.ptr(p1.b), _lib.ptr(p1.slope)), [_lib.ptr(v) for v in self._p23]
        if f16:
            lib.fr_pnet_conv1_band(0, self._fptr(frames), N, H, W, hs, ws, *p1w, None, _lib.ptr(xs), None, None, 0, self._s)
        else:
            self._dconv(None, p1, N, hs, ws, frames=frames, y_split=xs, y=x)
        if coarse > 0.0:
            lib.fr_pnet23_coarse_f16(_lib.ptr(x), _lib.ptr(xs), N, h, w, *p23, _lib.ptr(head), 2 if f16 else 0, lo, hi,
                                     _lib.ptr(self.refined_cells), _lib.ptr(wsp), wsp.numel() * 4, coarse, _lib.ptr(cws), cws.numel() * 4,
                                     _lib.ptr(self.visited_cells), self._s)
        else:
            lib.fr_pnet23_split_f16(_lib.ptr(x), _lib.ptr(xs), N, h, w, *p23, _lib.ptr(head),
                                    (1 if (self.p23_all_heads or trace is not None) else 0) | (2 if f16 else 0), lo, hi,
                                    _lib.ptr(self.refined_cells), _lib.ptr(wsp), wsp.numel() * 4, self._s)
        keep = None
        if f16:
            nt = lib.fr_pnet_band_tiles_count(N, h, w)
            tbuf, tiles = self._i32(1 + (nt + 31) // 32), self._i32(nt)
            lib.fr_pnet_band_tiles(_lib.ptr(wsp), N, h, w, _lib.ptr(tbuf), _lib.ptr(tiles), self._s)
            lib.fr_pnet_conv1_band(1, self._fptr(frames), N, H, W, hs, ws, *p1w, _lib.ptr(x), None, _lib.ptr(tiles), _lib.ptr(tbuf), nt, self._s)
            lib.fr_pnet_finish_levels((_lib.PnetLevel * 1)(entry), 1, N, *p23, cand[1], cand[2], lo, _lib.ptr(self.refined_cells), self._s)
            t.update(tbuf=tbuf, tiles=tiles)
            keep = (x, xs, head, wsp, tbuf, tiles, t["bc"])
        if self.level_tensors is not None:
            self.level_tensors.append(t)
        return head, h - 4, w - 4, t["bc"], wsp, lo, keep

    def pnet_level(self, frames, scale, trace=None, cand=None):
        N, H, W, _ = frames.shape
        geo = _level_geo(H, W, scale)
        fused = bool(self.fused_pnet) and N <= _frames32(*geo[2:])
        band = bool(self.pnet_band and _is_batch(self, N, H, W) and trace is None)
        f16 = fused and cand is not None and _f16_conv1(self, band, *geo[2:])
        coarse = self.coarse_margin if self.coarse_p23 and band else 0.0
        head, hc, wc, _, dl, dl_min, keep = self._level(frames, scale, geo, fused, band, f16, trace, cand, coarse)
        self._tls.dl, self._tls.level_done, self._tls.keep = (dl, dl_min), keep is not None, keep
        return head, hc, wc

    def _pnet_pyramid(self, frames, plan, cand):
        N, H, W, _ = frames.shape
        lib, p1, nlev = self.lib, self.p1, len(plan.scales)
        lo, hi = self._band_logits(plan.band)
        lv = (_lib.PnetLevel * nlev)()
        keep, ntile, words, coarse = [], 0, 0, self._coarse(plan.coarse)
        for li, (s, geo, f16) in enumerate(zip(plan.scales, plan.geo, plan.f16)):
            t, lv[li] = self._level_buffers(N, s, geo, plan.band, f16, [c[li] for c in cand], coarse)
            keep.append(t)
            if f16:
                nt = lib.fr_pnet_band_tiles_count(N, t["h"], t["w"])
                ntile, words = ntile + nt, words + (nt + 31) // 32
        p1w, p23 = (_lib.ptr(p1.w), _lib.ptr(p1.b), _lib.ptr(p1.slope)), [_lib.ptr(t) for t in self._p23]
        lib.fr_pnet_pyramid_conv1(0, self._fptr(frames), N, H, W, lv, nlev, *p1w, None, None, 0, self._s)
        if coarse > 0.0:
            cws = (ctypes.c_void_p * nlev)(*[t["cws"].data_ptr() for t in keep])
            lib.fr_pnet_pyramid_p23_coarse(lv, nlev, N, *p23, 0, lo, hi, coarse, cws, _lib.ptr(self.visited_cells), self._s)
        else:
            lib.fr_pnet_pyramid_p23(lv, nlev, N, *p23, 1 if self.p23_all_heads else 0, lo, hi, self._s)
        if ntile:
            tbuf, tiles = self._i32(1 + words), self._i32(ntile)
            lib.fr_pnet_pyramid_band_tiles(lv, nlev, N, _lib.ptr(tbuf), _lib.ptr(tiles), self._s)
            lib.fr_pnet_pyramid_conv1(1, self._fptr(frames), N, H, W, lv, nlev, *p1w, _lib.ptr(tiles), _lib.ptr(tbuf), ntile, self._s)
            keep[0].update(tbuf=tbuf, tiles=tiles)
        lib.fr_pnet_finish_levels(lv, nlev, N, *p23, self.thresholds[0], self.cap_scale, lo, _lib.ptr(self.refined_cells), self._s)
        if self.level_tensors is not None:
            self.level_tensors.extend(keep)

    @contextlib.contextmanager
    def _forked(self, main, n, events=None):
        note = self.lib.note
        sides = self._sides.setdefault(main.cuda_stream, [])
        while len(sides) < n:
            sides.append(torch.cuda.Stream(device=self.device))
        sides = sides[:n]
        if events is None:
            for side in sides:
                side.wait_stream(main)
        else:
            events[0].record(main)
            note(8, events[0].cuda_event, main.cuda_stream)
            for side in sides:
                side.wait_event(events[0])
                note(9, side.cuda_stream, events[0].cuda_event)
        yield sides
        if events is None:
            for side in sides:
                main.wait_stream(side)
        else:
            for side, ev in zip(sides, events[1:]):
                ev.record(side)
                note(8, ev.cuda_event, side.cuda_stream)
                main.wait_event(ev)
                note(9, main.cuda_stream, ev.cuda_event)
        self._s = ctypes.c_void_p(main.cuda_stream)

    def _pnet_levels(self, frames, plan, trace, cand):
        N, lib, t0, cs = plan.N, self.lib, self.thresholds[0], self.cap_scale
        events = (self._tls.rec or {}).get("events")
        forked = events is not None or not plan.solo
        main, keep = torch.cuda.current_stream(), []
        with (self._forked(main, len(events) - 1 if events else plan.nside, events) if forked else contextlib.nullcontext()) as sides:
            for li, s in enumerate(plan.scales):
                stream = sides[(li - 1) % len(sides)] if forked and li else main
                with (contextlib.nullcontext() if plan.solo else torch.cuda.stream(stream)):
                    if forked:
                        self._s = ctypes.c_void_p(stream.cuda_stream)
                    lcand = [c[li] for c in cand]
                    head, hc, wc, bc, dl, dl_min, done = self._level(
                        frames, s, plan.geo[li], plan.fused[li], plan.band, plan.f16[li], trace,
                        (float(s), t0, cs, *lcand) if plan.batch and trace is None else None, plan.coarse)
                    prob = self._f32(N, hc, wc) if trace is not None else None
                    if done is not None:
                        keep.append(done)
                    else:
                        lib.fr_pnet_candidates(_lib.ptr(head), N, hc, wc, float(s), t0, cs, *[_lib.ptr(c) for c in lcand], _lib.ptr(bc),
                                               _lib.ptr(prob), _lib.ptr(dl), dl_min, self._s)
                    if trace is not None:
                        trace.setdefault("pnet_head", []).append(head)
                        trace.setdefault("pnet_prob", []).append(prob)
        for grp in keep:
            for t in grp:
                t.record_stream(main)

    def _stage1(self, frames, plan, trace):
        N, nlev, cs, ksz = plan.N, len(plan.scales), self.cap_scale, self.keep_scale
        lb, ls, lr, lc = self._f32(nlev, N, cs, 4), self._f32(nlev, N, cs), self._f32(nlev, N, cs, 4), self._i32(nlev, N)
        kb, ks, ka, kc = self._f32(nlev, N, ksz, 4), self._f32(nlev, N, ksz), self._f32(nlev, N, ksz, 4), self._i32(nlev, N)
        if self.level_tensors is not None:
            del self.level_tensors[:]
        if plan.pyramid:
            self._pnet_pyramid(frames, plan, (lb, ls, lr, lc))
        else:
            self._pnet_levels(frames, plan, trace, (lb, ls, lr, lc))
        self._mark("pnet")
        if self.level_tensors is not None:
            self.level_tensors.append(dict(cand=(lb, ls, lr, lc)))
        self._nms(lb, ls, lr, 4, lc, nlev * N, 1, cs, 0, 0.5, 0, ksz, out=(kb, ks, ka, kc))
        b1, s1, a1, c1 = self._nms(kb, ks, ka, 4, kc, N, nlev, ksz, 1, 0.7, 0, self.cap_p)
        self.lib.fr_box_refine(_lib.ptr(b1), _lib.ptr(a1), 4, _lib.ptr(c1), N, self.cap_p, 0, self._s)
        self._mark("stage1_nms")
        if trace is not None:
            trace.update(stage1_boxes=b1, stage1_scores=s1, stage1_counts=c1)
        return b1, s1, a1, c1

    def crop_conv1(self, net, frames, boxes, counts, cap):
        N, H, W, _ = frames.shape
        t = _RO[net]
        w, b, s = getattr(self, t.w1)
        y = self._f32(N * cap, t.map1[0], t.map1[0], t.map1[1])
        self.lib.fr_crop_conv1_f32(net, self._fptr(frames), N, H, W, _lib.ptr(boxes), _lib.ptr(counts), cap, _lib.ptr(w),
                                   _lib.ptr(b), _lib.ptr(s), _lib.ptr(y), self._s)
        return y

    def crop_conv12_split(self, net, frames, boxes, counts, cap):
        N, H, W, _ = frames.shape
        t = _RO[net]
        (w1, b1, s1), (w2, b2, s2) = getattr(self, t.w1), getattr(self, t.w2)
        xs = self._new((N * cap, t.map1[0] ** 2, 128), torch.uint8)
        self.lib.fr_crop_conv1_split(net, self._fptr(frames), N, H, W, _lib.ptr(boxes), _lib.ptr(counts), cap, _lib.ptr(w1),
                                     _lib.ptr(b1), _lib.ptr(s1), _lib.ptr(xs), 1 if self.split_conv1 else 0, self._s)
        y = self._f32(N * cap, t.map2[0], t.map2[0], t.map2[1])
        lc = self._i32(1)
        self.lib.fr_ro_conv2_split(net, _lib.ptr(xs), _lib.ptr(w2), _lib.ptr(b2), _lib.ptr(s2), _lib.ptr(y), N * cap,
                                   _lib.ptr(counts), cap, _lib.ptr(lc), self._s)
        return y, lc

    def exact_pass(self, net, frames, boxes, counts, cap, head, thr, lc):
        N, H, W, _ = frames.shape
        t = _RO[net]
        w1, b1, s1 = getattr(self, t.w1)
        lcap, nh = self.ro_list_cap[net], head.shape[1]
        lst = self._i32(lcap)
        self.lib.fr_ro_margin_list(_lib.ptr(head), nh, _lib.ptr(counts), N, cap, math.log(thr / (1.0 - thr)), self.ro_margin,
                                   _lib.ptr(lst), _lib.ptr(lc), lcap, self._s)
        x1 = self._f32(lcap, t.map1[0], t.map1[0], t.map1[1])
        self.lib.fr_crop_conv1_list_f32(net, self._fptr(frames), N, H, W, _lib.ptr(boxes), cap, _lib.ptr(lst), _lib.ptr(lc), lcap,
                                        _lib.ptr(w1), _lib.ptr(b1), _lib.ptr(s1), _lib.ptr(x1), self._s)
        exact = getattr(self, t.name)(None, lcap, lc, lcap, x1=x1)
        self.lib.fr_ro_scatter_rows(_lib.ptr(exact), _lib.ptr(lst), _lib.ptr(lc), lcap, nh, _lib.ptr(head), self._s)
        self._tls.__dict__.setdefault("ro_lists", {})[net] = lc
        self._tls.path["exact_lists"].append((net, lcap))
        self._tls.exact_counters.append(lc)

    @property
    def _ro_lists(self):
        return getattr(self._tls, "ro_lists", {})

    def exact_lists(self):
        path = getattr(self._tls, "path", None)
        if not path:
            return []
        torch.cuda.synchronize(self.device)
        return [{"net": _RO[net].name, "count": int(lc[0]), "cap": cap}
                for (net, cap), lc in zip(path["exact_lists"], self._tls.exact_counters)]

    def exact_list_overflow(self):
        return sorted({e["net"] for e in self.exact_lists() if e["count"] > e["cap"]}, key=("rnet", "onet").index)

    def _net(self, t, x, B, counts, cap, x1, x2):
        k = dict(counts=counts, cap=cap)
        layers = [getattr(self, n) for n in t.layers]
        if x2 is not None:
            x, h, w = x2, t.map2[0], t.map2[0]
        else:
            x, h, w = (x1, t.map1[0], t.map1[0]) if x1 is not None else self._dconv(x, layers[0], B, t.crop, t.crop, **k)
            x, h, w = self._dconv(x, layers[1], B, h, w, **k)
        for c in layers[2:-1]:
            if x2 is not None:
                h, w = c.out_hw(h, w)
                x = self._gemm_split(c.layer, x, B, (h, w, c.cout), counts, cap)
            else:
                x, h, w = self._dconv(x, c, B, h, w, **k)
        x, _, _ = self._dconv(x, layers[-1], B, 1, 1, **k)
        return x.reshape(B, t.nhead)

    def rnet(self, x, B, counts=None, cap=0, x1=None, x2=None):
        return self._net(_RO[0], x, B, counts, cap, x1, x2)

    def onet(self, x, B, counts=None, cap=0, x1=None, x2=None):
        return self._net(_RO[1], x, B, counts, cap, x1, x2)

    def _refine_stage(self, net, frames, boxes, counts, plan, trace, out=None):
        t = _RO[net]
        N, H, W, _ = frames.shape
        lib, run, thr, crops = self.lib, getattr(self, t.name), self.thresholds[1 + net], None
        cap, cap_out = getattr(self, t.cap_in), getattr(self, t.cap_out)
        if plan.split:
            y, lc = self.crop_conv12_split(net, frames, boxes, counts, cap)
            head = run(None, N * cap, counts, cap, x2=y)
            self.exact_pass(net, frames, boxes, counts, cap, head, thr, lc)
        elif self.fused_crop and trace is None:
            head = run(None, N * cap, counts, cap, x1=self.crop_conv1(net, frames, boxes, counts, cap))
        else:
            crops = self._f32(N * cap, t.crop, t.crop, 4)
            lib.fr_crop_resize_norm(self._fptr(frames), N, H, W, _lib.ptr(boxes), _lib.ptr(counts), cap, t.crop, _lib.ptr(crops), self._s)
            head = run(crops, N * cap, counts, cap)
        sb, ss, sa, sc = self._f32(N, cap, 4), self._f32(N, cap), self._f32(N, cap, t.naux), self._i32(N)
        prob = self._f32(N, cap) if trace is not None else None
        lib.fr_stage_select(_lib.ptr(boxes), _lib.ptr(head), t.nhead, _lib.ptr(counts), N, cap, thr, _lib.ptr(sb), _lib.ptr(ss),
                            _lib.ptr(sa), t.naux, _lib.ptr(sc), _lib.ptr(prob), self._s)
        if net == 0:
            res = self._nms(sb, ss, sa, t.naux, sc, N, 1, cap, 0, 0.7, 0, cap_out)
            lib.fr_box_refine(_lib.ptr(res[0]), _lib.ptr(res[2]), t.naux, _lib.ptr(res[3]), N, cap_out, t.refine, self._s)
        else:
            lib.fr_box_refine(_lib.ptr(sb), _lib.ptr(sa), t.naux, _lib.ptr(sc), N, cap, t.refine, self._s)
            self._tls.cache = None
            res = self._nms(sb, ss, sa, t.naux, sc, N, 1, cap, 0, 0.7, 1, cap_out, out=out, results=True)
        self._mark("stage%d" % (2 + net))
        if trace is not None:
            trace.update({t.name + "_head": head, t.name + "_prob": prob})
            if net == 0:
                trace.update(rnet_crops=crops, stage2_boxes=res[0], stage2_scores=res[1], stage2_counts=res[3])
        return res

    def _mark(self, name):
        if self.phase_marks is not None:
            e = torch.cuda.Event(enable_timing=True)
            e.record()
            self.phase_marks.append((name, e))

    def _begin(self, frames, plan):
        tls = self._tls
        tls.rec = None
        if not plan.cache:
            return None
        caches, seqs = tls.__dict__.setdefault("caches", {}), tls.__dict__.setdefault("seqs", {})
        key = (*frames.shape[:3], torch.cuda.current_stream().cuda_stream)
        if key not in caches and len(caches) >= 4:
            old_key = next(iter(caches))
            caches.pop(old_key); seqs.pop(old_key, None)
        known = key in caches
        tls.cache = [caches.setdefault(key, []), 0]
        cfg = (self.fused_pnet, self.fused_crop, self.p23_all_heads, self.thresholds, self.refine_margin,
               self.cap_scale, self.keep_scale, self.cap_p, self.cap_r, self.cap_o, self.minsize, self.factor, self.coarse_p23, self.coarse_margin)
        seq = seqs.get(key)
        if seq is not None and (not plan.recorder or seq["cfg"] != cfg):
            seqs.pop(key)
            seq = None
        if seq is not None:
            tls.cache = None
            return seq
        tls.rec = {"key": key, "cfg": cfg, "events": None}
        if plan.recorder and known:
            self.lib.start_recording()
            tls.rec["events"] = [torch.cuda.Event() for _ in range(1 + min(4, max(1, len(plan.scales) - 1)))]

    def _end(self, frames, outs):
        tls = self._tls
        rec, tls.rec = tls.rec, None
        if rec is None:
            return
        if rec["events"] is not None:
            calls = self.lib.stop_recording()
            if calls and not tls.cache_grew:
                seq = self._make_sequence(calls, frames, outs, rec["cfg"])
                if seq is not None:
                    seq["events"] = rec["events"]
                    tls.seqs[rec["key"]] = seq
        if tls.cache_grew:
            tls.seqs.pop(rec["key"], None)

    def detect_batch(self, frames, trace=None, level_streams=None, _out=None):
        assert frames.dtype == torch.uint8 and frames.dim() == 4 and frames.shape[3] == 3 and frames.is_contiguous()
        N, H, W, _ = frames.shape
        with torch.cuda.device(self.device):
            plan = detect_plan(N, H, W, self, trace is not None, level_streams, _out is not None, torch.cuda.is_current_stream_capturing())
            if _out is None:
                self._tls.path = {"frames": N, "batch": plan.batch, "chunks": max(1, len(plan.chunks)), "fused_levels": 0, "band_levels": 0, "coarse_levels": 0,
                                  "pconv1_mfma_levels": [], "unfused_levels": 0, "split_ro": False, "exact_lists": []}
                self._tls.exact_counters = []
            if plan.chunks:
                out = tuple(torch.empty(sh, dtype=dt, device=self.device) for sh, dt in (
                    ((N, self.cap_o, 4), torch.float32), ((N, self.cap_o), torch.float32), ((N, self.cap_o, 14), torch.float32), ((N,), torch.int32)))
                for n0, n1 in plan.chunks:
                    self.detect_batch(frames[n0:n1], None, level_streams, _out=tuple(t[n0:n1] for t in out))
                return out[0], out[1], out[2][..., 4:14].unflatten(-1, (5, 2)), out[3]
            self._s = _lib.stream_ptr()
            self._tls.cache, self._tls.cache_grew = None, False
            self.lib.stop_recording()
            self._mark("start")
            if not plan.scales:
                z = torch.zeros((N, self.cap_o, 14), dtype=torch.float32, device=self.device)
                return (z[..., :4].contiguous(), z[..., 0].contiguous(), z[..., 4:14].unflatten(-1, (5, 2)),
                        torch.zeros(N, dtype=torch.int32, device=self.device))
            assert len(plan.scales) * self.keep_scale <= 4096, "too many pyramid levels for the merged NMS list"
            seq = self._begin(frames, plan)
            if seq is not None:
                return self._replay(seq, frames)
            b1, _, _, c1 = self._stage1(frames, plan, trace)
            self._tls.path["split_ro"] = plan.split
            b2, _, _, c2 = self._refine_stage(0, frames, b1, c1, plan, trace)
            b3, s3, a3, c3 = self._refine_stage(1, frames, b2, c2, plan, trace, out=_out)
            self._end(frames, (b3, s3, a3, c3))
            return b3, s3, a3[..., 4:14].unflatten(-1, (5, 2)), c3

    def _make_sequence(self, calls, frames, outs, cfg):
        log = logging.getLogger(__name__)
        arr = (_lib.Call * len(calls))()
        want = {"frame": frames.data_ptr(), **{"out%d" % i: t.data_ptr() for i, t in enumerate(outs)}}
        fpos, opos = [], [[] for _ in outs]
        for k, (fid, slots, roles) in enumerate(calls):
            arr[k].fn, arr[k].nargs = fid, len(slots)
            for i, v in enumerate(slots):
                arr[k].a[i] = v
            tagged = dict(roles)
            for i, role in roles:
                if slots[i] != want[role]:
                    log.warning("MTCNNHIP: recorded call %d: slot %d carries the role '%s' but holds another tensor; call list refused", k, i, role)
                    return None
                (fpos if role == "frame" else opos[int(role[3:])]).append((k, i))
            if fid < 8:
                for i, v in enumerate(slots):
                    if i not in tagged and v in want.values():
                        log.warning("MTCNNHIP: recorded call %d: slot %d holds a patched tensor without its role; call list refused", k, i)
                        return None
        if not fpos or not all(opos):
            log.warning("MTCNNHIP: the recorded call list does not mention the frame and every result tensor; refused")
            return None
        return {"arr": arr, "n": len(calls), "fpos": fpos, "opos": opos, "cfg": cfg,
                "meta": [(tuple(t.shape), t.dtype) for t in outs]}

    def _replay(self, seq, frames):
        arr = seq["arr"]
        outs = [torch.empty(shape, dtype=dtype, device=self.device) for shape, dtype in seq["meta"]]
        fptr = frames.data_ptr()
        for k, i in seq["fpos"]:
            arr[k].a[i] = fptr
        for t, pos in zip(outs, seq["opos"]):
            p = t.data_ptr()
            for k, i in pos:
                arr[k].a[i] = p
        self.lib.fr_detect_sequence(arr, seq["n"])
        b3, s3, a3, c3 = outs
        return b3, s3, a3[..., 4:14].unflatten(-1, (5, 2)), c3
```

### include/frhip.h

```cpp
#ifndef FRHIP_H
#define FRHIP_H
#include <stddef.h>
#include <stdint.h>
#ifdef __cplusplus
extern "C" {
#endif

#define FR_OK 0
#define FR_E_INVALID (-1)
#define FR_E_LAUNCH (-2)
#define FR_E_NODEVICE (-3)

typedef void* fr_stream_t;

#define FR_ABI_VERSION 106
int fr_version(void);
const char* fr_last_error_string(void);
int fr_device_count(void);

int fr_l2norm_rows_f32(const float* x, float* out, int rows, int dim, fr_stream_t stream);

size_t fr_gallery_match_workspace(int F, int64_t N);
int fr_gallery_match_f32(const float* Q, const float* G, int F, int64_t N, int D,
                         int64_t row_offset, int64_t* out_idx, float* out_score,
                         void* workspace, size_t workspace_bytes, const int32_t* seg_counts, int seg_len,
                         fr_stream_t stream);
int fr_gallery_match_view_f32(const float* Q, const float* G, const int64_t* view, int F, int64_t Nview, int D,
                              int64_t* out_idx, float* out_score, void* workspace, size_t workspace_bytes,
                              fr_stream_t stream);
int fr_gallery_update_rows_f32(float* G, const int64_t* slots, const float* rows, int n, int D, int normalise,
                               fr_stream_t stream);
#define FR_TOPK 4
#define FR_TOPK8 8
#define FR_F8_SCALE 256.0f
size_t fr_gallery_match_f16_workspace(int F, int64_t N);
int fr_gallery_match_f16(const float* Q, const void* G16, const float* G32, int F, int64_t N, int D,
                         int64_t row_offset, int64_t* out_idx, float* out_score,
                         void* workspace, size_t workspace_bytes, const int32_t* seg_counts, int seg_len,
                         fr_stream_t stream);
size_t fr_gallery_match_f8_workspace(int F, int64_t N);
int fr_gallery_match_f8(const float* Q, const void* G8, const float* G32, int F, int64_t N, int D,
                        int64_t row_offset, int64_t* out_idx, float* out_score,
                        void* workspace, size_t workspace_bytes, const int32_t* seg_counts, int seg_len,
                        fr_stream_t stream);
#define FR_TOPK_MAX 16
size_t fr_gallery_topk_workspace(int F, int64_t N, int K);
int fr_gallery_topk_f32(const float* Q, const float* G, int F, int64_t N, int D, int K, int64_t row_offset,
                        int64_t* out_idx , float* out_score , void* workspace,
                        size_t workspace_bytes, const int32_t* seg_counts, int seg_len, fr_stream_t stream);
int fr_gallery_topk_view_f32(const float* Q, const float* G, const int64_t* view, int F, int64_t Nview, int D,
                             int K, int64_t* out_idx, float* out_score, void* workspace,
                             size_t workspace_bytes, fr_stream_t stream);
#define FR_SHADOW_F16 1
#define FR_SHADOW_F8 2
int fr_gallery_update_rows_shadow(float* G, void* shadow, int shadow_kind, const int64_t* slots, const float* rows,
                                  int n, int D, int normalise, fr_stream_t stream);
size_t fr_gallery_match_view_f16_workspace(int F, int64_t Nview);
int fr_gallery_match_view_f16(const float* Q, const void* S16, const float* G32, const int64_t* view, int F,
                              int64_t Nview, int64_t capacity, int D, int64_t* out_idx, float* out_score,
                              void* workspace, size_t workspace_bytes, fr_stream_t stream);
size_t fr_gallery_match_view_f8_workspace(int F, int64_t Nview);
int fr_gallery_match_view_f8(const float* Q, const void* S8, const float* G32, const int64_t* view, int F,
                             int64_t Nview, int64_t capacity, int D, int64_t* out_idx, float* out_score,
                             void* workspace, size_t workspace_bytes, fr_stream_t stream);
size_t fr_gallery_topk_f16_workspace(int F, int64_t N, int K);
int fr_gallery_topk_f16(const float* Q, const void* G16, const float* G32, int F, int64_t N, int D, int K,
                        int64_t row_offset, const float* gmax, int64_t* out_idx, float* out_score, int32_t* flags,
                        void* workspace, size_t workspace_bytes, const int32_t* seg_counts, int seg_len,
                        fr_stream_t stream);
size_t fr_gallery_topk_view_f16_workspace(int F, int64_t Nview, int K);
int fr_gallery_topk_view_f16(const float* Q, const void* S16, const float* G32, const int64_t* view, int F,
                             int64_t Nview, int64_t capacity, int D, int K, const float* gmax, int64_t* out_idx,
                             float* out_score, int32_t* flags, void* workspace, size_t workspace_bytes,
                             fr_stream_t stream);
int fr_gallery_topk_view_masked_f32(const float* Q, const float* G, const int64_t* view, int F, int64_t Nview, int D,
                                    int K, int64_t* out_idx, float* out_score, void* workspace,
                                    size_t workspace_bytes, const int32_t* mask, fr_stream_t stream);
int fr_gallery_gmax_update(const float* G, const int64_t* slots, int64_t n, int D, float* gmax, fr_stream_t stream);
size_t fr_gallery_match_grouped_workspace(int ngroups, int64_t max_view_len);
int fr_gallery_match_grouped_f32(const float* Q, const float* G, const int64_t* views, const int64_t* gtab,
                                 const int32_t* qmap, int F, int ngroups, int64_t max_view_len, int64_t capacity, int D,
                                 int64_t* out_idx, float* out_score, void* workspace, size_t workspace_bytes,
                                 const int32_t* seg_counts, int seg_len, fr_stream_t stream);
size_t fr_gallery_topk_grouped_workspace(int ngroups, int64_t max_view_len, int K);
int fr_gallery_topk_grouped_f32(const float* Q, const float* G, const int64_t* views, const int64_t* gtab,
                                const int32_t* qmap, int F, int ngroups, int64_t max_view_len, int64_t capacity, int D,
                                int K, int64_t* out_idx , float* out_score , void* workspace,
                                size_t workspace_bytes, const int32_t* seg_counts, int seg_len, fr_stream_t stream);
int fr_f32_to_f8(const float* x, void* out, int64_t n, fr_stream_t stream);
int fr_f32_to_f16(const float* x, void* out, int64_t n, fr_stream_t stream);
int fr_match_decide(const int64_t* idx, const float* score, int F, float thr, float unknown_thr,
                    int32_t* decision, fr_stream_t stream);


int fr_match_pack_candidates(const int64_t* idx, const float* score, int n, int32_t* cand, fr_stream_t stream);
int fr_match_reduce_shards(const int32_t* cand_all, int R, int n, int q0, int F, int64_t* out_idx,
                           float* out_score, fr_stream_t stream);
int fr_match_reduce_shards_topk(const int32_t* cand_all, int R, int n, int K, int q0, int F,
                                int64_t* out_idx, float* out_score, fr_stream_t stream);
int fr_exchange_pack_queries(const float* Q, int F, int q_max, int D, float* send, fr_stream_t stream);
int fr_exchange_counts(const float* gathered, int R, int q_max, int D, int32_t* counts, fr_stream_t stream);


int fr_gallery_first_above_f32(const float* Q, const float* G, int F, int64_t N, int D, float thr,
                               int inclusive, int64_t row_offset, int64_t* out_idx, float* out_score,
                               void* workspace, size_t workspace_bytes, fr_stream_t stream);
int fr_cosine_matrix_f32(const float* A, const float* B, int F, int N, int D, float* out,
                         fr_stream_t stream);
int fr_mean_rows_f32(const float* x, int K, int D, float* out, fr_stream_t stream);
#define FR_UNKNOWN_N 0
#define FR_UNKNOWN_OVERFLOW 1
#define FR_UNKNOWN_HEADER 4
#define FR_UNKNOWN_STATE_INTS(capacity) (FR_UNKNOWN_HEADER + 3 * (capacity))
int fr_unknown_assign_batch_f32(const float* E, const int32_t* take, int F, int D, float thr, float* avg, float* hist,
                                int32_t* state, int capacity, int depth, int32_t* out_cluster, int32_t* out_new,
                                int32_t* out_count, fr_stream_t stream);

int fr_gallery_first_above_blocked_f32(const float* Q, const float* G, const int64_t* view, const int32_t* take, int F,
                                       int64_t N, int D, float thr, int inclusive, int64_t row_offset, int64_t* out_idx,
                                       float* out_score, void* workspace, size_t workspace_bytes, fr_stream_t stream);
#define FR_ENROL_DONE 0
#define FR_ENROL_NO_FACE 1
#define FR_ENROL_DIFFERENT 2
#define FR_ENROL_DUPLICATE 3
#define FR_ENROL_MAX_POSES 8
#define FR_ENROL_MAX_JOBS 256
size_t fr_enrol_batch_workspace(int J, int64_t N);
int fr_enrol_batch_f32(const float* E, const float* bbox, int S, const int32_t* img_first, const int32_t* img_count, int I,
                       const int32_t* job_first, int J, int max_poses, int D, const float* G, const int64_t* view, int64_t N,
                       float sim_thr, float dup_thr, int32_t* status, int32_t* pair, int32_t* face, float* avg, float* row,
                       int64_t* dup_pos, float* dup_score, void* workspace, size_t workspace_bytes, fr_stream_t stream);
#define FR_PAIRS_OVERFLOW 1
#define FR_PAIRS_NONFINITE 2
size_t fr_gallery_pairs_workspace(int64_t N, int64_t capacity);
int fr_gallery_pairs_above_f16(const float* G32, const int64_t* view, int64_t N, int D, float thr, int inclusive,
                               int64_t capacity, int max_ranges, int64_t* out_key, float* out_score, int32_t* out_counts,
                               void* workspace, size_t workspace_bytes, fr_stream_t stream);

typedef struct {
    const void* x; const void* w; void* y;
    const float* bias; const float* slope; const void* residual;
    float* out_f32_partial;
    int B, H, W, Cin, Cout, KH, KW, stride, pad, Ho, Wo;
    int bias_mode; int splitk;
    const void* x2; int C2;
} fr_conv_args;
int fr_conv_nhwc_f16(const fr_conv_args* args, fr_stream_t stream);
typedef struct {
    const void* x8; const void* w8; void* y16; void* y8;
    const float* oscale; const float* bias; const float* slope; const void* residual;
    int B, H, W, Cin, Cout, bias_mode;
    float y8_mul;
    const float* y8_sub;
} fr_conv_f8_args;
int fr_conv_nhwc_f8(const fr_conv_f8_args* args, fr_stream_t stream);
int fr_quantize_f16_f8(const void* x16, void* out8, int64_t n, float mul, fr_stream_t stream);
int fr_quantize_f16_f8_centred(const void* x16, void* out8, int64_t n, int C, const float* sub, float mul,
                               fr_stream_t stream);
size_t fr_conv_stage14_weight_bytes(int nconv);
int fr_conv_stage14_pack(const void* w, void* out, fr_stream_t stream);
int fr_conv_stage14_f16(const void* x, void* y, const void* wstream, const float* params, int B, int nblocks,
                        fr_stream_t stream);
size_t fr_conv_stage28_weight_bytes(int nconv);
int fr_conv_stage28_pack(const void* w, void* out, fr_stream_t stream);
int fr_conv_stage28_f16(void* x, void* mid, const void* wstream, const float* params, int B, int nblocks, fr_stream_t stream);
size_t fr_conv_walk64_weight_bytes(int Cout);
int fr_conv_walk64_pack(const void* w, void* out, int Cout, fr_stream_t stream);
int fr_conv_walk64_f16(const void* x, const void* wstream, void* y, const float* bias, int bias_mode, const float* slope,
                       const void* residual, int B, int HW, int Cout, fr_stream_t stream);
size_t fr_conv_stage14_f8_weight_bytes(int nconv);
size_t fr_conv_stage14_f8_param_floats(void);
int fr_conv_stage14_f8_pack(const void* w8, void* out, fr_stream_t stream);
int fr_conv_stage14_f8(const void* x8, const void* x16, void* y16, const void* wstream, const float* params, int B,
                       int nblocks, fr_stream_t stream);
int fr_gptq_round_e4m3(const double* W, const double* U, const float* sw, float* Q, int rows, int K, fr_stream_t stream);
int fr_conv_splitk_epilogue(const float* partial, int splitk, int M, int Cout, int Ho, int Wo,
                            const float* bias, int bias_mode, const float* slope, const void* residual,
                            void* y, fr_stream_t stream);
int fr_conv_inblock_f16(const fr_conv_args* args, fr_stream_t stream);
typedef struct {
    int kind;
    fr_conv_args args;
} fr_conv_step;
int fr_conv_sequence(const fr_conv_step* steps, int nsteps, fr_stream_t stream);
int fr_fc_reduce_l2norm(const float* partial, int splitk, int B, int dim, const float* bias,
                        float* embedding, float* normed, fr_stream_t stream);


int fr_warp_affine_5pt(const uint8_t* frames, int nframes, int H, int W, const float* kps,
                       const int32_t* frame_idx, const int32_t* count, int F, int size,
                       void* out_f16_nhwc8, uint8_t* out_u8_bgr, float* M_out, fr_stream_t stream);

int fr_warp_affine_5pt_slots(const uint8_t* frames, int nframes, int H, int W, const float* kps,
                             const int32_t* counts, int cap, int size, void* out_f16_nhwc8,
                             fr_stream_t stream);

typedef struct {
    const uint8_t* data;
    int32_t H, W, nh, nw;
    int32_t reserved[2];
} fr_frame_ref;
int fr_warp_affine_5pt_refs(const fr_frame_ref* refs, int nframes, const float* kps, const int32_t* frame_idx,
                            const int32_t* count, int F, int size, void* out_f16_nhwc8, uint8_t* out_u8_bgr,
                            float* M_out, fr_stream_t stream);
int fr_warp_affine_5pt_slots_refs(const fr_frame_ref* refs, int nframes, const float* kps, const int32_t* counts,
                                  int cap, int size, void* out_f16_nhwc8, fr_stream_t stream);

int fr_pyramid_resize_norm(const uint8_t* frames, int nframes, int H, int W, int hs, int ws,
                           float* out, fr_stream_t stream);
int fr_dconv_f32(const float* x, const float* w, const float* bias, const float* slope, float* y,
                 int B, int H, int W, int Cin, int Cout, int CoutP, int KH, int KW, int pool2,
                 const float* head_w, const float* head_b, int nhead, fr_stream_t stream);
int fr_dconv_mfma_f32(int layer, const float* x, const float* w, const float* bias, const float* slope,
                      float* y, int B, int H, int W, const float* head_w, const float* head_b,
                      const uint8_t* frames, int FH, int FW, const int32_t* counts, int cap, void* y_split,
                      fr_stream_t stream);
int fr_crop_conv1_f32(int net, const uint8_t* frames, int nframes, int H, int W, const float* boxes,
                      const int32_t* counts, int cap, const float* w, const float* bias, const float* slope,
                      float* y, fr_stream_t stream);
#define FR_RC1_BATCH_SHAPE 16
int fr_crop_conv1_split(int net, const uint8_t* frames, int nframes, int H, int W, const float* boxes,
                        const int32_t* counts, int cap, const float* w, const float* bias, const float* slope,
                        void* y_split, int conv_f16, fr_stream_t stream);
int fr_crop_conv1_list_f32(int net, const uint8_t* frames, int nframes, int H, int W, const float* boxes, int cap,
                           const int32_t* list, const int32_t* list_count, int list_cap, const float* w,
                           const float* bias, const float* slope, float* y, fr_stream_t stream);
int fr_ro_conv2_split(int net, const void* x_split, const float* w, const float* bias, const float* slope, float* y,
                      int nslots, const int32_t* counts, int cap, int32_t* zero_word, fr_stream_t stream);
size_t fr_ro_gemm_weight_bytes(int layer);
int fr_ro_gemm_pack(int layer, const float* w, void* out, fr_stream_t stream);
int fr_ro_gemm_split(int layer, const float* x, const void* w_packed, const float* bias, const float* slope, float* y,
                     int nslots, const int32_t* counts, int cap, fr_stream_t stream);
int fr_ro_margin_list(const float* head, int nhead, const int32_t* counts, int nframes, int cap, float logit_thr,
                      float margin, int32_t* list, int32_t* list_count, int list_cap, fr_stream_t stream);
int fr_ro_scatter_rows(const float* src, const int32_t* list, const int32_t* list_count, int list_cap, int ncols,
                       float* dst, fr_stream_t stream);
size_t fr_pnet23_workspace_bytes(int B, int H1, int W1);
int fr_pnet23_split_f16(const float* x1, const void* x1s, int B, int H1, int W1, const float* w2, const float* b2, const float* s2,
                        const float* w3, const float* b3, const float* s3, const float* hw, const float* hb,
                        float* head, int all_heads, float refine_logit_thr, float refine_band_hi, int32_t* refined_count,
                        void* workspace, size_t workspace_bytes, fr_stream_t stream);
size_t fr_pnet23_coarse_workspace_bytes(int B, int H1, int W1);
int fr_pnet23_coarse_f16(const float* x1, const void* x1s, int B, int H1, int W1, const float* w2, const float* b2, const float* s2,
                         const float* w3, const float* b3, const float* s3, const float* hw, const float* hb,
                         float* head, int all_heads, float refine_logit_thr, float refine_band_hi, int32_t* refined_count,
                         void* workspace, size_t workspace_bytes, float coarse_margin, void* coarse, size_t coarse_bytes,
                         int32_t* visited_count, fr_stream_t stream);
int fr_maxpool_f32(const float* x, float* y, int B, int H, int W, int C, int k, int stride,
                   fr_stream_t stream);
int fr_pnet_candidates(const float* head, int nframes, int hc, int wc, float scale, float thr, int cap,
                       float* boxes, float* scores, float* regs, int32_t* counts,
                       int32_t* block_counts, float* prob_out, const float* dl, float dl_min, fr_stream_t stream);
int fr_sort_nms(const float* boxes, const float* scores, const float* aux, int naux,
                const int32_t* counts, int L, int nseg, int seg_cap, int seg_major, float thr, int mode,
                int max_keep,
                float* boxes_out, float* scores_out, float* aux_out, int32_t* counts_out,
                int cap_out, fr_stream_t stream);
int fr_box_refine(float* boxes, const float* aux, int naux, const int32_t* counts, int L, int cap,
                  int mode, fr_stream_t stream);
int fr_crop_resize_norm(const uint8_t* frames, int nframes, int H, int W, const float* boxes,
                        const int32_t* counts, int cap, int size, float* out, fr_stream_t stream);
int fr_stage_select(const float* boxes, const float* head, int nh, const int32_t* counts, int L, int cap,
                    float thr, float* boxes_out, float* scores_out, float* aux_out, int naux,
                    int32_t* counts_out, float* prob_out, fr_stream_t stream);

int fr_pnet_conv1_band(int mode, const uint8_t* frames, int B, int FH, int FW, int H, int W, const float* w, const float* bias,
                       const float* slope, float* y, void* y_split, const int32_t* list, const int32_t* list_count, int list_cap,
                       fr_stream_t stream);
size_t fr_pnet_band_tiles_count(int B, int H1, int W1);
int fr_pnet_band_tiles(const void* workspace, int B, int H1, int W1, int32_t* tbuf, int32_t* tiles, fr_stream_t stream);
typedef struct {
    const float* x1; float* head; void* workspace;
    int H1, W1; float scale;
    float* boxes; float* scores; float* regs; int32_t* counts; int32_t* block_counts;
    void* x1s;
    int hs, ws;
    int f16;
} fr_pnet_level;
int fr_pnet_finish_levels(const fr_pnet_level* levels, int nlevels, int nframes, const float* w2, const float* b2,
                          const float* s2, const float* w3, const float* b3, const float* s3, const float* hw,
                          const float* hb, float thr, int cap, float dl_min, int32_t* refined_count, fr_stream_t stream);
int fr_pnet_pyramid_conv1(int mode, const uint8_t* frames, int B, int FH, int FW, const fr_pnet_level* levels, int nlevels,
                          const float* w, const float* bias, const float* slope, const int32_t* list, const int32_t* list_count,
                          int list_cap, fr_stream_t stream);
int fr_pnet_pyramid_p23(const fr_pnet_level* levels, int nlevels, int nframes, const float* w2, const float* b2, const float* s2,
                        const float* w3, const float* b3, const float* s3, const float* hw, const float* hb, int all_heads,
                        float refine_logit_thr, float refine_band_hi, fr_stream_t stream);
int fr_pnet_pyramid_band_tiles(const fr_pnet_level* levels, int nlevels, int nframes, int32_t* tbuf, int32_t* tiles, fr_stream_t stream);
int fr_pnet_pyramid_p23_coarse(const fr_pnet_level* levels, int nlevels, int nframes, const float* w2, const float* b2, const float* s2,
                               const float* w3, const float* b3, const float* s3, const float* hw, const float* hb, int all_heads,
                               float refine_logit_thr, float refine_band_hi, float coarse_margin, void* const* coarse,
                               int32_t* visited_count, fr_stream_t stream);

int fr_letterbox_u8(const fr_frame_ref* refs, int nframes, uint8_t* canvas, int dh, int dw, fr_stream_t stream);
int fr_detections_unscale(float* boxes, float* kps, const int32_t* counts, const float* det_scale, int nframes, int cap,
                          fr_stream_t stream);

#define FR_YUV_NV12 0
#define FR_YUV_I420 1
int fr_yuv420_to_bgr_u8(const uint8_t* src, uint8_t* dst, int N, int H, int W, int layout, int y_off, int cy, int cub, int cug,
                        int cvg, int cvr, fr_stream_t stream);
int fr_yuv420_to_bgr_refs_u8(const fr_frame_ref* dst_refs, const uint8_t* const* src_ptrs, int nframes, int layout, int y_off,
                             int cy, int cub, int cug, int cvg, int cvr, fr_stream_t stream);

int fr_frame_activity_u8(const uint8_t* frames, int N, int H, int W, const int32_t* slot, int S, uint8_t* grid, int32_t* geom,
                         int32_t* idle, int C, uint8_t* cur, int32_t* changed, int32_t* active, int thr, int min_cells,
                         int max_idle, fr_stream_t stream);
int fr_frame_activity_refs_u8(const fr_frame_ref* refs, int nframes, const int32_t* slot, int S, uint8_t* grid, int32_t* geom,
                              int32_t* idle, int C, uint8_t* cur, int32_t* changed, int32_t* active, int thr, int min_cells,
                              int max_idle, fr_stream_t stream);

#define FR_HUD_K 16
#define FR_HUD_MAX_CAP 64
#define FR_HUD_MAX_CHARS 64
int fr_hud_draw_u8(uint8_t* frames, int N, int H, int W, const int32_t* counts, int cap, const int32_t* faces,
                   const uint8_t* text, int max_chars, const uint8_t* font, int scale, fr_stream_t stream);
int fr_hud_draw_refs_u8(const fr_frame_ref* refs, int nframes, const int32_t* counts, int cap, const int32_t* faces,
                        const uint8_t* text, int max_chars, const uint8_t* font, int scale, fr_stream_t stream);

int fr_track_associate_f32(const float* boxes, const int32_t* counts, const int32_t* slot, int N, int cap, int S, int T,
                           float* tbox, int32_t* tstate, int32_t* next_id, float iou_thr, int max_reuse, int max_misses,
                           int32_t* entry, int32_t* need, int32_t* tid, fr_stream_t stream);
int fr_track_commit_f32(const int32_t* entry, const int32_t* need, const int32_t* slot, const int32_t* counts, int N, int cap,
                        int S, int T, float* bank, float* emb, float* normed, fr_stream_t stream);

int fr_track_resolve_quality_i32(const int32_t* entry, const int32_t* need, const int32_t* tid, const int32_t* verdict,
                                 const int32_t* slot, const int32_t* counts, int N, int cap, int S, int T, int32_t* tstate,
                                 int32_t* tqual, int max_age, int32_t* action, int32_t* need2, int32_t* entry2,
                                 fr_stream_t stream);

int fr_track_fuse_f32(const int32_t* entry, const int32_t* need, const int32_t* tid, const int32_t* slot, const int32_t* counts,
                      const float* normed, int N, int cap, int S, int T, int K, float join_thr, float* tring, int32_t* ttmpl,
                      float* tmean, float* query, int32_t* shots, int32_t* event, fr_stream_t stream);

int fr_face_quality_f16(const void* crops, const float* kps, const int32_t* slot_counts, int cap, int S, int32_t* qi, float* qf,
                        int32_t* verdict, float min_eye2, int mean_lo, int mean_hi, int contrast_min, int sharp_min, int clip_max,
                        float yaw_max, float pitch_lo, float pitch_hi, fr_stream_t stream);

size_t fr_det_conv_weight_halves(int Cin, int cout_packed, int K);
int fr_det_conv_f16(const void* x, const void* w, const float* bias, const void* residual, void* y, int N, int H, int W,
                    int Cin, int cout_packed, int K, int stride, int pad, int Ho, int Wo, int cout_store, int ldo,
                    int relu, int out_f32, int tile, fr_stream_t stream);
int fr_det_conv_act_f16(const void* x, const void* w, const float* bias, const float* slope, const void* residual, void* y,
                        int N, int H, int W, int Cin, int cout_packed, int K, int stride, int pad, int Ho, int Wo,
                        int cout_store, int ldo, int act, int out_f32, int tile, fr_stream_t stream);
int fr_dw_conv_f16(const void* x, const void* w, const float* bias, const float* slope, void* y, int N, int H, int W, int C, int K,
                   int stride, int pad, int Ho, int Wo, int act, fr_stream_t stream);
int fr_det_input_f16(const uint8_t* canvas, void* y, int N, int H, int W, fr_stream_t stream);
int fr_det_pool_f16(const void* x, void* y, int N, int H, int W, int C, int Ho, int Wo, int kind, int k, int stride,
                    int pad, fr_stream_t stream);
int fr_det_upsample_add_f16(const void* coarse, const void* lateral, void* y, int N, int H, int W, int C, int up,
                            fr_stream_t stream);
int fr_scrfd_decode(const float* score, const float* bbox, const float* kps, int nframes, int Hl, int Wl, int A, int stride,
                    int level, float logit_thr, const float* det_scale, int cap, float* boxes, float* scores, float* aux,
                    int32_t* counts, fr_stream_t stream);

enum { FR_FN_DCONV_MFMA = 1, FR_FN_PNET23 = 2, FR_FN_PNET_CANDIDATES = 3, FR_FN_SORT_NMS = 4, FR_FN_BOX_REFINE = 5,
       FR_FN_CROP_CONV1 = 6, FR_FN_STAGE_SELECT = 7,
       FR_FN_EVENT_RECORD = 8 , FR_FN_STREAM_WAIT = 9  };
typedef struct {
    int32_t fn; int32_t nargs;
    uint64_t a[22];
} fr_call;
int fr_detect_sequence(const fr_call* calls, int ncalls);

#ifdef __cplusplus
}
#endif
#endif
```

Baseline: 27040.

## Add tall 16-row tiles to the coarse PNet conv2/conv3 pass

Adds a templated 16-row form of the fused coarse PNet conv2+conv3+head kernel. It pairs vertically adjacent 8-row tiles so a block processes one taller window, sharing the halo rows between the two tiles and cutting how many times the conv1 activations are loaded. Python picks 16-row tiles per pyramid level when each block would otherwise handle at least two tiles, using a new launcher that selects the tile height per level. In exchange it uses more LDS per block, which may lower occupancy, and it adds more complex tile-indexing logic.

```diff
diff --git a/facerecognition_infrenceengine_amd/_lib.py b/facerecognition_infrenceengine_amd/_lib.py
--- a/facerecognition_infrenceengine_amd/_lib.py
+++ b/facerecognition_infrenceengine_amd/_lib.py
@@ -168,7 +168,10 @@
     "fr_pnet_band_tiles": (_I, [_P, _I, _I, _I, _P, _P, _P]),
     "fr_pnet23_coarse_workspace_bytes": (_Z, [_I, _I, _I]),
     "fr_pnet23_coarse_f16": (_I, [_P, _P, _I, _I, _I, _P, _P, _P, _P, _P, _P, _P, _P, _P, _I, _F, _F, _P, _P, _Z, _F, _P, _Z, _P, _P]),
+    "fr_pnet23_coarse_tiles_f16": (_I, [_P, _P, _I, _I, _I, _P, _P, _P, _P, _P, _P, _P, _P, _P, _I, _F, _F, _P, _P, _Z, _F, _P, _Z, _I, _P, _P]),
     "fr_pnet_pyramid_p23_coarse": (_I, [C.POINTER(PnetLevel), _I, _I, _P, _P, _P, _P, _P, _P, _P, _P, _I, _F, _F, _F, C.POINTER(_P), _P, _P]),
+    "fr_pnet_pyramid_p23_coarse_tiles": (_I, [C.POINTER(PnetLevel), _I, _I, _P, _P, _P, _P, _P, _P, _P, _P, _I, _F, _F, _F, C.POINTER(_P),
+                                              C.POINTER(C.c_int32), _P, _P]),
     "fr_pnet_finish_levels": (_I, [C.POINTER(PnetLevel), _I, _I, _P, _P, _P, _P, _P, _P, _P, _P, _F, _I, _F, _P, _P]),
     "fr_pnet_pyramid_conv1": (_I, [_I, _P, _I, _I, _I, C.POINTER(PnetLevel), _I, _P, _P, _P, _P, _P, _I, _P]),
     "fr_pnet_pyramid_p23": (_I, [C.POINTER(PnetLevel), _I, _I, _P, _P, _P, _P, _P, _P, _P, _P, _I, _F, _F, _P]),
diff --git a/facerecognition_infrenceengine_amd/csrc/pnet_fused.hip b/facerecognition_infrenceengine_amd/csrc/pnet_fused.hip
--- a/facerecognition_infrenceengine_amd/csrc/pnet_fused.hip
+++ b/facerecognition_infrenceengine_amd/csrc/pnet_fused.hip
@@ -49,13 +49,40 @@
     for (int e = tid; e < 8; e += NT) cst[96 + e] = e < 6 ? a.hb[e] : 0.f;
 }
 
-template <bool COARSE>
+__device__ __forceinline__ void p23_tall_item(const P23Args& a, const int vb, const int vgrid, const int it, int& n, int& ty0, int& tx0,
+                                              int& rows, int& next) {
+    const int k = a.seg_cap / (P23_RH * P23_RW), paired = k & ~1;
+    n = ty0 = tx0 = rows = 0; next = it + 1;
+    if (it >= k) return;
+    const int u = it < paired ? 2 * ((it >> 1) * vgrid + vb) + (it & 1) : paired * vgrid + vb;
+    if (u >= a.ntiles) return;
+    const int prow = a.tiles_y >> 1, npair = a.B * prow * a.tiles_x;
+    if (u < 2 * npair) {
+        const int p = u >> 1, per = prow * a.tiles_x;
+        n = p / per;
+        const int rem = p - n * per;
+        ty0 = (2 * (rem / a.tiles_x) + (u & 1)) * P23_RH; tx0 = (rem % a.tiles_x) * P23_RW;
+        if (it < paired && !(u & 1)) { rows = 2 * P23_RH; next = it + 2; }
+        else rows = P23_RH;
+    } else {
+        const int j = u - 2 * npair;
+        n = j / a.tiles_x; ty0 = (a.tiles_y - 1) * P23_RH; tx0 = (j - n * a.tiles_x) * P23_RW; rows = P23_RH;
+    }
+}
+
+template <bool COARSE, int RH = P23_RH>
 __device__ __forceinline__ void pnet23_body(const P23Args& a, const int vb, const int vgrid, char* lds) {
 #if defined(__HIP_DEVICE_COMPILE__)
+    static_assert(RH == P23_RH || (COARSE && RH == 16), "only the coarse pass has a tall form");
     constexpr int NP = COARSE ? 1 : 2;
+    constexpr int X1PX = (RH + 4) * P23_X1W, X2PX = (RH + 2) * P23_X2W, X2T = (X2PX + 15) / 16;
+    constexpr int NPC = (X1PX + 31) / 32;
+    constexpr int X1PL = NPC * 1024, X2PL = X2PX * 32;
+    constexpr int NT2 = (X2T + 7) / 8, NT3 = RH / 4;
+    static_assert(X1PL == P23_X1PL || RH != P23_RH, "the 8-row form's planes");
     char* x1t = lds;
-    char* x2t = x1t + NP * P23_X1PL;
-    char* wf = x2t + NP * P23_X2PL;
+    char* x2t = x1t + NP * X1PL;
+    char* wf = x2t + NP * X2PL;
     float* cst = reinterpret_cast<float*>(wf + NP * 15 * 1024);
     int* lcnt = reinterpret_cast<int*>(cst + 104);
     const int tid = threadIdx.x, lane = tid & 63, wave = tid >> 6;
@@ -75,26 +102,37 @@
     }
 
     __amdgpu_buffer_rsrc_t xrs = buffer_rsrc(a.x1s, a.x1s_bytes);
-    constexpr int NPIECE = 14 * NP, NI = (NPIECE + 7) / 8;
+    constexpr int NPIECE = NPC * NP, NI = (NPIECE + 7) / 8;
     int wy[NI], wx[NI], wc[NI];
 #pragma unroll
     for (int i = 0; i < NI; ++i) {
-        const int j = wave + 8 * i, pl = j >= 14 ? 1 : 0;
-        const int p = (j - 14 * pl) * 32 + (lane >> 1);
-        wy[i] = p < P23_X1PX ? p / P23_X1W : 1 << 20; wx[i] = p % P23_X1W;
+        const int j = wave + 8 * i, pl = j >= NPC ? 1 : 0;
+        const int p = (j - NPC * pl) * 32 + (lane >> 1);
+        wy[i] = p < X1PX ? p / P23_X1W : 1 << 20; wx[i] = p % P23_X1W;
         wc[i] = pl * 32 + (lane & 1) * 16;
     }
-    auto issue_window = [&](int tile) {
-        const int per = a.tiles_x * a.tiles_y;
-        const int n = tile / per, rem = tile - n * per;
-        const int ty0 = (rem / a.tiles_x) * P23_RH, tx0 = (rem % a.tiles_x) * P23_RW;
+    auto item = [&](int it, int& n, int& ty0, int& tx0, int& rows, int& next) {
+        if constexpr (RH == P23_RH) {
+            const int per = a.tiles_x * a.tiles_y;
+            n = it / per;
+            const int rem = it - n * per;
+            ty0 = (rem / a.tiles_x) * P23_RH; tx0 = (rem % a.tiles_x) * P23_RW;
+            rows = it < a.ntiles ? P23_RH : 0; next = it + vgrid;
+        } else {
+            p23_tall_item(a, vb, vgrid, it, n, ty0, tx0, rows, next);
+        }
+    };
+    auto issue_window = [&](int it) {
+        int n, ty0, tx0, rows, next;
+        item(it, n, ty0, tx0, rows, next);
+        if (RH != P23_RH && !rows) return;
 #pragma unroll
         for (int i = 0; i < NI; ++i) {
             const int j = wave + 8 * i;
             if (j < NPIECE) {
                 const int gy = ty0 + wy[i], gx = tx0 + wx[i];
                 const unsigned off = (gy < a.H1 && gx < a.W1) ? (unsigned)(((n * a.H1 + gy) * a.W1 + gx) * 64 + wc[i]) : 0x80000000u;
-                __builtin_amdgcn_raw_ptr_buffer_load_lds(xrs, (lds_ptr_t)(x1t + (j >= 14 ? P23_X1PL + (j - 14) * 1024 : j * 1024)), 16, off, 0, 0, 0);
+                __builtin_amdgcn_raw_ptr_buffer_load_lds(xrs, (lds_ptr_t)(x1t + (j >= NPC ? X1PL + (j - NPC) * 1024 : j * 1024)), 16, off, 0, 0, 0);
             }
         }
     };
@@ -108,21 +146,23 @@
         split_f16(w, hwh, hwl, j);
     }
     (void)hwl;
-    issue_window(vb);
-    for (int tile = vb; tile < a.ntiles; tile += vgrid) {
-        const int per = a.tiles_x * a.tiles_y;
-        const int n = tile / per, rem = tile - n * per;
-        const int ty0 = (rem / a.tiles_x) * P23_RH, tx0 = (rem % a.tiles_x) * P23_RW;
+    int tile = RH == P23_RH ? vb : 0;
+    issue_window(tile);
+    for (;;) {
+        int n, ty0, tx0, rows, next;
+        item(tile, n, ty0, tx0, rows, next);
+        if (!rows) break;
         asm volatile("s_waitcnt vmcnt(0)" ::: "memory");
         __syncthreads();
         {
-            const int t0 = wave < 6 ? wave * 3 : 18 + (wave - 6) * 2, nt = wave < 6 ? 3 : 2;
-            int pb[3];
-            float4v acc[3];
-#pragma unroll
-            for (int t = 0; t < 3; ++t) {
+            constexpr int FULL = X2T - 8 * (NT2 - 1);
+            const int t0 = wave < FULL ? wave * NT2 : FULL * NT2 + (wave - FULL) * (NT2 - 1), nt = wave < FULL ? NT2 : NT2 - 1;
+            int pb[NT2];
+            float4v acc[NT2];
+#pragma unroll
+            for (int t = 0; t < NT2; ++t) {
                 int q = (t0 + t) * 16 + fr;
-                if (q >= P23_X2PX) q = 0;
+                if (q >= X2PX) q = 0;
                 pb[t] = ((q / P23_X2W) * P23_X1W + q % P23_X2W) * 32;
                 acc[t] = float4v{0.f, 0.f, 0.f, 0.f};
             }
@@ -131,7 +171,7 @@
                 const half8 ahi = *reinterpret_cast<const half8*>(wf + ((ks * NP + 0) * 64 + lane) * 16);
                 if constexpr (COARSE) {
 #pragma unroll
-                    for (int t = 0; t < 3; ++t) {
+                    for (int t = 0; t < NT2; ++t) {
                         if (t < nt) {
                             const half8 bhi = *reinterpret_cast<const half8*>(x1t + (pb[t] + off2[ks]));
                             acc[t] = __builtin_amdgcn_mfma_f32_16x16x32_f16(ahi, bhi, acc[t], 0, 0, 0);
@@ -140,11 +180,11 @@
                 } else {
                     const half8 alo = *reinterpret_cast<const half8*>(wf + ((ks * 2 + 1) * 64 + lane) * 16);
 #pragma unroll
-                    for (int t = 0; t < 3; ++t) {
+                    for (int t = 0; t < NT2; ++t) {
                         if (t < nt) {
                             const char* bp = x1t + (pb[t] + off2[ks]);
                             const half8 bhi = *reinterpret_cast<const half8*>(bp);
-                            const half8 blo = *reinterpret_cast<const half8*>(bp + P23_X1PL);
+                            const half8 blo = *reinterpret_cast<const half8*>(bp + X1PL);
                             acc[t] = __builtin_amdgcn_mfma_f32_16x16x32_f16(alo, bhi, acc[t], 0, 0, 0);
                             acc[t] = __builtin_amdgcn_mfma_f32_16x16x32_f16(ahi, blo, acc[t], 0, 0, 0);
                             acc[t] = __builtin_amdgcn_mfma_f32_16x16x32_f16(ahi, bhi, acc[t], 0, 0, 0);
@@ -154,9 +194,9 @@
             }
             const float4v bb = *reinterpret_cast<const float4v*>(cst + 4 * fq), ss = *reinterpret_cast<const float4v*>(cst + 16 + 4 * fq);
 #pragma unroll
-            for (int t = 0; t < 3; ++t) {
+            for (int t = 0; t < NT2; ++t) {
                 const int q = (t0 + t) * 16 + fr;
-                if (t < nt && q < P23_X2PX) {
+                if (t < nt && q < X2PX) {
                     float4v v = acc[t] + bb;
 #pragma unroll
                     for (int e = 0; e < 4; ++e) v[e] = __builtin_fmaf(fminf(v[e], 0.f), ss[e], v[e]);
@@ -171,19 +211,19 @@
 #pragma unroll
                         for (int e = 0; e < 4; ++e) split_f16(v[e], hi, lo, e);
                         *reinterpret_cast<half4*>(o) = hi;
-                        *reinterpret_cast<half4*>(o + P23_X2PL) = lo;
+                        *reinterpret_cast<half4*>(o + X2PL) = lo;
                     }
                 }
             }
         }
         __syncthreads();
-        if (tile + vgrid < a.ntiles) issue_window(tile + vgrid);
+        if (RH != P23_RH || next < a.ntiles) issue_window(next);
         {
-            int pb[2];
-            float4v acc[2][2];
-#pragma unroll
-            for (int t = 0; t < 2; ++t) {
-                const int q = (wave * 2 + t) * 16 + fr;
+            int pb[NT3];
+            float4v acc[NT3][2];
+#pragma unroll
+            for (int t = 0; t < NT3; ++t) {
+                const int q = (wave * NT3 + t) * 16 + fr;
                 pb[t] = ((q >> 5) * P23_X2W + (q & 31)) * 32;
                 acc[t][0] = acc[t][1] = float4v{0.f, 0.f, 0.f, 0.f};
             }
@@ -194,7 +234,7 @@
 #pragma unroll
                     for (int ct = 0; ct < 2; ++ct) ahi[ct] = *reinterpret_cast<const half8*>(wf + ((5 + ct * 5 + ks) * 64 + lane) * 16);
 #pragma unroll
-                    for (int t = 0; t < 2; ++t) {
+                    for (int t = 0; t < NT3; ++t) {
                         const half8 bhi = *reinterpret_cast<const half8*>(x2t + (pb[t] + off3[ks]));
 #pragma unroll
                         for (int ct = 0; ct < 2; ++ct) acc[t][ct] = __builtin_amdgcn_mfma_f32_16x16x32_f16(ahi[ct], bhi, acc[t][ct], 0, 0, 0);
@@ -208,10 +248,10 @@
                     alo[ct] = *reinterpret_cast<const half8*>(wf + (((5 + ct * 5 + ks) * 2 + 1) * 64 + lane) * 16);
                 }
 #pragma unroll
-                for (int t = 0; t < 2; ++t) {
+                for (int t = 0; t < NT3; ++t) {
                     const char* bp = x2t + (pb[t] + off3[ks]);
                     const half8 bhi = *reinterpret_cast<const half8*>(bp);
-                    const half8 blo = *reinterpret_cast<const half8*>(bp + P23_X2PL);
+                    const half8 blo = *reinterpret_cast<const half8*>(bp + X2PL);
 #pragma unroll
                     for (int ct = 0; ct < 2; ++ct) {
                         acc[t][ct] = __builtin_amdgcn_mfma_f32_16x16x32_f16(alo[ct], bhi, acc[t][ct], 0, 0, 0);
@@ -223,7 +263,7 @@
             const float4v b30 = *reinterpret_cast<const float4v*>(cst + 32 + 4 * fq), s30 = *reinterpret_cast<const float4v*>(cst + 64 + 4 * fq);
             const float4v b31 = *reinterpret_cast<const float4v*>(cst + 48 + 4 * fq), s31 = *reinterpret_cast<const float4v*>(cst + 80 + 4 * fq);
 #pragma unroll
-            for (int t = 0; t < 2; ++t) {
+            for (int t = 0; t < NT3; ++t) {
                 float4v v0 = acc[t][0] + b30, v1 = acc[t][1] + b31;
                 half8 bh, bl;
 #pragma unroll
@@ -239,9 +279,9 @@
                     d = __builtin_amdgcn_mfma_f32_16x16x32_f16(hwh, bl, d, 0, 0, 0);
                 }
                 d = __builtin_amdgcn_mfma_f32_16x16x32_f16(hwh, bh, d, 0, 0, 0);
-                const int q = (wave * 2 + t) * 16 + fr;
+                const int q = (wave * NT3 + t) * 16 + fr;
                 const int gy = ty0 + (q >> 5), gx = tx0 + (q & 31);
-                const bool inb = fq < 2 && gy < a.H3 && gx < a.W3;
+                const bool inb = fq < 2 && gy < a.H3 && gx < a.W3 && (RH == P23_RH || (q >> 5) < rows);
                 const size_t cell = ((size_t)n * a.H3 + gy) * a.W3 + gx;
                 const float4v hb4 = *reinterpret_cast<const float4v*>(cst + 96 + 4 * (fq & 1));
                 const float o0 = d[0] + hb4[0], o1 = d[1] + hb4[1];
@@ -265,6 +305,7 @@
                 }
             }
         }
+        tile = next;
     }
     __syncthreads();
     if (tid == 0) (COARSE ? a.ccounts : a.counts)[vb] = *lcnt;
@@ -319,6 +360,15 @@
     const int l = p23_find_level(t, (int)blockIdx.x);
     p23_set_level(a, t, c, l);
     pnet23_body<true>(a, (int)blockIdx.x - t.first[l], t.first[l + 1] - t.first[l], lds);
+}
+
+struct P23Tall { int rows[P23_MAXL]; };
+__global__ __launch_bounds__(P23_NT, 4) void pnet23_coarse_tall(P23Args a, P23Levels t, P23Coarse c, P23Tall r) {
+    extern __shared__ __attribute__((aligned(16))) char lds[];
+    const int l = p23_find_level(t, (int)blockIdx.x);
+    p23_set_level(a, t, c, l);
+    if (r.rows[l] == 2 * P23_RH) pnet23_body<true, 2 * P23_RH>(a, (int)blockIdx.x - t.first[l], t.first[l + 1] - t.first[l], lds);
+    else pnet23_body<true>(a, (int)blockIdx.x - t.first[l], t.first[l + 1] - t.first[l], lds);
 }
 
 #define P23R_NT 256
@@ -637,19 +687,20 @@
 
 constexpr size_t P23_LDS = (size_t)2 * P23_X1PL + (size_t)2 * P23_X2PL + 30 * 1024 + 108 * 4;
 constexpr size_t P23C_LDS = (size_t)P23_X1PL + (size_t)P23_X2PL + 15 * 1024 + 108 * 4;
+constexpr size_t P23T_LDS = (size_t)23 * 1024 + (size_t)(2 * P23_RH + 2) * P23_X2W * 32 + 15 * 1024 + 108 * 4;
 
 static int p23_level(const char* who, const float* x1, const void* x1s, int B, int H1, int W1, const float* w2, const float* b2,
                      const float* s2, const float* w3, const float* b3, const float* s3, const float* hw,
                      const float* hb, float* head, int all_heads, float refine_logit_thr, float refine_band_hi,
                      int32_t* refined_count, void* workspace, size_t workspace_bytes, float coarse_margin, void* coarse,
-                     size_t coarse_bytes, int32_t* visited_count, fr_stream_t stream);
+                     size_t coarse_bytes, int tile_rows, int32_t* visited_count, fr_stream_t stream);
 
 extern "C" int fr_pnet23_split_f16(const float* x1, const void* x1s, int B, int H1, int W1, const float* w2, const float* b2,
                                    const float* s2, const float* w3, const float* b3, const float* s3, const float* hw,
                                    const float* hb, float* head, int all_heads, float refine_logit_thr, float refine_band_hi,
                                    int32_t* refined_count, void* workspace, size_t workspace_bytes, fr_stream_t stream) {
     return p23_level("fr_pnet23_split_f16", x1, x1s, B, H1, W1, w2, b2, s2, w3, b3, s3, hw, hb, head, all_heads, refine_logit_thr,
-                     refine_band_hi, refined_count, workspace, workspace_bytes, 0.f, nullptr, 0, nullptr, stream);
+                     refine_band_hi, refined_count, workspace, workspace_bytes, 0.f, nullptr, 0, P23_RH, nullptr, stream);
 }
 
 extern "C" int fr_pnet23_coarse_f16(const float* x1, const void* x1s, int B, int H1, int W1, const float* w2, const float* b2,
@@ -660,14 +711,26 @@
     FR_REQUIRE(!(all_heads & 1), "fr_pnet23_coarse_f16: all_heads & 1 (the approximate heads of every cell) needs fr_pnet23_split_f16");
     FR_REQUIRE(coarse && coarse_margin >= 0.f, "fr_pnet23_coarse_f16: needs a coarse buffer and a margin >= 0");
     return p23_level("fr_pnet23_coarse_f16", x1, x1s, B, H1, W1, w2, b2, s2, w3, b3, s3, hw, hb, head, all_heads, refine_logit_thr,
-                     refine_band_hi, refined_count, workspace, workspace_bytes, coarse_margin, coarse, coarse_bytes, visited_count, stream);
+                     refine_band_hi, refined_count, workspace, workspace_bytes, coarse_margin, coarse, coarse_bytes, P23_RH, visited_count, stream);
+}
+
+extern "C" int fr_pnet23_coarse_tiles_f16(const float* x1, const void* x1s, int B, int H1, int W1, const float* w2, const float* b2,
+                                          const float* s2, const float* w3, const float* b3, const float* s3, const float* hw,
+                                          const float* hb, float* head, int all_heads, float refine_logit_thr, float refine_band_hi,
+                                          int32_t* refined_count, void* workspace, size_t workspace_bytes, float coarse_margin,
+                                          void* coarse, size_t coarse_bytes, int tile_rows, int32_t* visited_count, fr_stream_t stream) {
+    FR_REQUIRE(!(all_heads & 1), "fr_pnet23_coarse_tiles_f16: all_heads & 1 (the approximate heads of every cell) needs fr_pnet23_split_f16");
+    FR_REQUIRE(coarse && coarse_margin >= 0.f, "fr_pnet23_coarse_tiles_f16: needs a coarse buffer and a margin >= 0");
+    FR_REQUIRE(tile_rows == P23_RH || tile_rows == 2 * P23_RH, "fr_pnet23_coarse_tiles_f16: tile_rows must be %d or %d (got %d)", P23_RH, 2 * P23_RH, tile_rows);
+    return p23_level("fr_pnet23_coarse_tiles_f16", x1, x1s, B, H1, W1, w2, b2, s2, w3, b3, s3, hw, hb, head, all_heads, refine_logit_thr,
+                     refine_band_hi, refined_count, workspace, workspace_bytes, coarse_margin, coarse, coarse_bytes, tile_rows, visited_count, stream);
 }
 
 static int p23_level(const char* who, const float* x1, const void* x1s, int B, int H1, int W1, const float* w2, const float* b2,
                      const float* s2, const float* w3, const float* b3, const float* s3, const float* hw,
                      const float* hb, float* head, int all_heads, float refine_logit_thr, float refine_band_hi,
                      int32_t* refined_count, void* workspace, size_t workspace_bytes, float coarse_margin, void* coarse,
-                     size_t coarse_bytes, int32_t* visited_count, fr_stream_t stream) {
+                     size_t coarse_bytes, int tile_rows, int32_t* visited_count, fr_stream_t stream) {
     FR_REQUIRE(x1 && x1s && w2 && b2 && s2 && w3 && b3 && s3 && hw && hb && head, "%s: null pointer", who);
     FR_REQUIRE((int64_t)B * H1 * W1 * 64 < (1ll << 31), "%s: the split conv1 map must stay below 2 GiB (got %lld bytes)", who, (long long)B * H1 * W1 * 64);
     FR_REQUIRE(B > 0 && H1 >= 5 && W1 >= 5, "%s: the conv1 map must be at least 5x5 (got %dx%d)", who, H1, W1);
@@ -697,12 +760,21 @@
         static FrDevLatch latch0, latch1;
         if (!fr_raise_lds(reinterpret_cast<const void*>(pnet23_coarse_f16), P23C_LDS, latch0) ||
             !fr_raise_lds(reinterpret_cast<const void*>(pnet23_reeval_levels), P23R_LDS, latch1)) { fr_set_error("fr_pnet23_coarse_f16: cannot raise dynamic LDS"); return FR_E_LAUNCH; }
-        pnet23_coarse_f16<<<grid, P23_NT, P23C_LDS, s>>>(a);
-        FR_CHECK_LAUNCH("pnet23_coarse_f16");
         P23Levels t{};
         P23Coarse c{};
         t.nlevels = 1; t.x1s[0] = a.x1s; t.head[0] = head; t.dl[0] = a.dl; t.H1[0] = H1; t.W1[0] = W1; t.seg_cap[0] = seg_cap;
         t.first[0] = 0; t.first[1] = grid; c.buf[0] = a.ccounts;
+        if (tile_rows != P23_RH) {
+            static FrDevLatch latch2;
+            P23Tall tall{};
+            tall.rows[0] = tile_rows;
+            if (!fr_raise_lds(reinterpret_cast<const void*>(pnet23_coarse_tall), P23T_LDS, latch2)) { fr_set_error("%s: cannot raise dynamic LDS", who); return FR_E_LAUNCH; }
+            pnet23_coarse_tall<<<grid, P23_NT, P23T_LDS, s>>>(a, t, c, tall);
+            FR_CHECK_LAUNCH("pnet23_coarse_tall");
+        } else {
+            pnet23_coarse_f16<<<grid, P23_NT, P23C_LDS, s>>>(a);
+            FR_CHECK_LAUNCH("pnet23_coarse_f16");
+        }
         pnet23_reeval_levels<<<p23_reeval_grid(grid), P23R_NT, P23R_LDS, s>>>(a, t, c);
         FR_CHECK_LAUNCH("pnet23_reeval_levels");
     } else {
@@ -798,13 +870,13 @@
 static int p23_pyramid(const char* who, const fr_pnet_level* levels, int nlevels, int nframes, const float* w2, const float* b2,
                        const float* s2, const float* w3, const float* b3, const float* s3, const float* hw,
                        const float* hb, int all_heads, float refine_logit_thr, float refine_band_hi, float coarse_margin,
-                       void* const* coarse, int32_t* visited_count, fr_stream_t stream);
+                       void* const* coarse, const int32_t* tile_rows, int32_t* visited_count, fr_stream_t stream);
 
 extern "C" int fr_pnet_pyramid_p23(const fr_pnet_level* levels, int nlevels, int nframes, const float* w2, const float* b2,
                                    const float* s2, const float* w3, const float* b3, const float* s3, const float* hw,
                                    const float* hb, int all_heads, float refine_logit_thr, float refine_band_hi, fr_stream_t stream) {
     return p23_pyramid("fr_pnet_pyramid_p23", levels, nlevels, nframes, w2, b2, s2, w3, b3, s3, hw, hb, all_heads, refine_logit_thr,
-                       refine_band_hi, 0.f, nullptr, nullptr, stream);
+                       refine_band_hi, 0.f, nullptr, nullptr, nullptr, stream);
 }
 
 extern "C" int fr_pnet_pyramid_p23_coarse(const fr_pnet_level* levels, int nlevels, int nframes, const float* w2, const float* b2,
@@ -814,21 +886,40 @@
     FR_REQUIRE(!(all_heads & 1), "fr_pnet_pyramid_p23_coarse: all_heads & 1 (the approximate heads of every cell) needs fr_pnet_pyramid_p23");
     FR_REQUIRE(coarse && coarse_margin >= 0.f, "fr_pnet_pyramid_p23_coarse: needs the coarse buffers and a margin >= 0");
     return p23_pyramid("fr_pnet_pyramid_p23_coarse", levels, nlevels, nframes, w2, b2, s2, w3, b3, s3, hw, hb, all_heads, refine_logit_thr,
-                       refine_band_hi, coarse_margin, coarse, visited_count, stream);
+                       refine_band_hi, coarse_margin, coarse, nullptr, visited_count, stream);
+}
+
+extern "C" int fr_pnet_pyramid_p23_coarse_tiles(const fr_pnet_level* levels, int nlevels, int nframes, const float* w2, const float* b2,
+                                                const float* s2, const float* w3, const float* b3, const float* s3, const float* hw,
+                                                const float* hb, int all_heads, float refine_logit_thr, float refine_band_hi,
+                                                float coarse_margin, void* const* coarse, const int32_t* tile_rows,
+                                                int32_t* visited_count, fr_stream_t stream) {
+    FR_REQUIRE(!(all_heads & 1), "fr_pnet_pyramid_p23_coarse_tiles: all_heads & 1 (the approximate heads of every cell) needs fr_pnet_pyramid_p23");
+    FR_REQUIRE(coarse && coarse_margin >= 0.f, "fr_pnet_pyramid_p23_coarse_tiles: needs the coarse buffers and a margin >= 0");
+    FR_REQUIRE(tile_rows, "fr_pnet_pyramid_p23_coarse_tiles: needs the levels' tile heights");
+    return p23_pyramid("fr_pnet_pyramid_p23_coarse_tiles", levels, nlevels, nframes, w2, b2, s2, w3, b3, s3, hw, hb, all_heads,
+                       refine_logit_thr, refine_band_hi, coarse_margin, coarse, tile_rows, visited_count, stream);
 }
 
 static int p23_pyramid(const char* who, const fr_pnet_level* levels, int nlevels, int nframes, const float* w2, const float* b2,
                        const float* s2, const float* w3, const float* b3, const float* s3, const float* hw,
                        const float* hb, int all_heads, float refine_logit_thr, float refine_band_hi, float coarse_margin,
-                       void* const* coarse, int32_t* visited_count, fr_stream_t stream) {
+                       void* const* coarse, const int32_t* tile_rows, int32_t* visited_count, fr_stream_t stream) {
     FR_REQUIRE(levels && nlevels > 0 && nlevels <= P23_MAXL && nframes > 0, "%s: 1 .. %d levels", who, P23_MAXL);
     FR_REQUIRE(w2 && b2 && s2 && w3 && b3 && s3 && hw && hb, "%s: null pointer", who);
     P23Levels t;
     P23Coarse c{};
+    P23Tall tall{};
+    bool any_tall = false;
     t.nlevels = nlevels;
     long long total = 0;
     for (int l = 0; l < nlevels; ++l) {
         const fr_pnet_level& L = levels[l];
+        if (tile_rows) {
+            FR_REQUIRE(tile_rows[l] == P23_RH || tile_rows[l] == 2 * P23_RH, "%s: level %d: tile_rows must be %d or %d (got %d)", who, l, P23_RH, 2 * P23_RH, tile_rows[l]);
+            tall.rows[l] = tile_rows[l];
+            any_tall = any_tall || tile_rows[l] != P23_RH;
+        }
         if (coarse) {
             FR_REQUIRE(coarse[l], "%s: level %d: no coarse buffer", who, l);
             c.buf[l] = reinterpret_cast<int*>(coarse[l]);
@@ -851,8 +942,15 @@
         static FrDevLatch latch0, latch1;
         if (!fr_raise_lds(reinterpret_cast<const void*>(pnet23_coarse_levels), P23C_LDS, latch0) ||
             !fr_raise_lds(reinterpret_cast<const void*>(pnet23_reeval_levels), P23R_LDS, latch1)) { fr_set_error("fr_pnet_pyramid_p23_coarse: cannot raise dynamic LDS"); return FR_E_LAUNCH; }
-        pnet23_coarse_levels<<<(unsigned)total, P23_NT, P23C_LDS, fr_stream(stream)>>>(a, t, c);
-        FR_CHECK_LAUNCH("pnet23_coarse_levels");
+        if (any_tall) {
+            static FrDevLatch latch2;
+            if (!fr_raise_lds(reinterpret_cast<const void*>(pnet23_coarse_tall), P23T_LDS, latch2)) { fr_set_error("%s: cannot raise dynamic LDS", who); return FR_E_LAUNCH; }
+            pnet23_coarse_tall<<<(unsigned)total, P23_NT, P23T_LDS, fr_stream(stream)>>>(a, t, c, tall);
+            FR_CHECK_LAUNCH("pnet23_coarse_tall");
+        } else {
+            pnet23_coarse_levels<<<(unsigned)total, P23_NT, P23C_LDS, fr_stream(stream)>>>(a, t, c);
+            FR_CHECK_LAUNCH("pnet23_coarse_levels");
+        }
         pnet23_reeval_levels<<<p23_reeval_grid(total), P23R_NT, P23R_LDS, fr_stream(stream)>>>(a, t, c);
         FR_CHECK_LAUNCH("pnet23_reeval_levels");
         return FR_OK;
diff --git a/facerecognition_infrenceengine_amd/mtcnn.py b/facerecognition_infrenceengine_amd/mtcnn.py
--- a/facerecognition_infrenceengine_amd/mtcnn.py
+++ b/facerecognition_infrenceengine_amd/mtcnn.py
@@ -124,6 +124,8 @@
     coarse_p23 = True
     coarse_margin = 0.05
     visited_cells = None
+    coarse_tall = True
+    coarse_tall_min_tiles = 2
 
     def __init__(self, minsize=20, factor=0.709, fused_pnet=True, batch_min_pixels=None):
         self.minsize, self.factor = minsize, factor
@@ -162,6 +164,11 @@
 
 def _frames32(h, w):
     return (2 ** 31 - 1) // (h * w * 64)
+
+
+def _coarse_tile_rows(cfg, N, h, w):
+    tiles = N * -(-(h - 4) // 8) * -(-(w - 4) // 32)
+    return 16 if cfg.coarse_tall and -(-tiles // min(tiles, 512)) >= cfg.coarse_tall_min_tiles else 8
 
 
 def _f16_conv1(cfg, band, h, w):
@@ -402,7 +409,11 @@
             lib.fr_pnet_conv1_band(0, self._fptr(frames), N, H, W, hs, ws, *p1w, None, _lib.ptr(xs), None, None, 0, self._s)
         else:
             self._dconv(None, p1, N, hs, ws, frames=frames, y_split=xs, y=x)
-        if coarse > 0.0:
+        if coarse > 0.0 and _coarse_tile_rows(self, N, h, w) > 8:
+            lib.fr_pnet23_coarse_tiles_f16(_lib.ptr(x), _lib.ptr(xs), N, h, w, *p23, _lib.ptr(head), 2 if f16 else 0, lo, hi,
+                                           _lib.ptr(self.refined_cells), _lib.ptr(wsp), wsp.numel() * 4, coarse, _lib.ptr(cws), cws.numel() * 4,
+                                           16, _lib.ptr(self.visited_cells), self._s)
+        elif coarse > 0.0:
             lib.fr_pnet23_coarse_f16(_lib.ptr(x), _lib.ptr(xs), N, h, w, *p23, _lib.ptr(head), 2 if f16 else 0, lo, hi,
                                      _lib.ptr(self.refined_cells), _lib.ptr(wsp), wsp.numel() * 4, coarse, _lib.ptr(cws), cws.numel() * 4,
                                      _lib.ptr(self.visited_cells), self._s)
@@ -450,7 +461,12 @@
         lib.fr_pnet_pyramid_conv1(0, self._fptr(frames), N, H, W, lv, nlev, *p1w, None, None, 0, self._s)
         if coarse > 0.0:
             cws = (ctypes.c_void_p * nlev)(*[t["cws"].data_ptr() for t in keep])
-            lib.fr_pnet_pyramid_p23_coarse(lv, nlev, N, *p23, 0, lo, hi, coarse, cws, _lib.ptr(self.visited_cells), self._s)
+            rows = [_coarse_tile_rows(self, N, t["h"], t["w"]) for t in keep]
+            if max(rows) > 8:
+                lib.fr_pnet_pyramid_p23_coarse_tiles(lv, nlev, N, *p23, 0, lo, hi, coarse, cws, (ctypes.c_int32 * nlev)(*rows),
+                                                     _lib.ptr(self.visited_cells), self._s)
+            else:
+                lib.fr_pnet_pyramid_p23_coarse(lv, nlev, N, *p23, 0, lo, hi, coarse, cws, _lib.ptr(self.visited_cells), self._s)
         else:
             lib.fr_pnet_pyramid_p23(lv, nlev, N, *p23, 1 if self.p23_all_heads else 0, lo, hi, self._s)
         if ntile:
diff --git a/include/frhip.h b/include/frhip.h
--- a/include/frhip.h
+++ b/include/frhip.h
@@ -246,6 +246,11 @@
                          float* head, int all_heads, float refine_logit_thr, float refine_band_hi, int32_t* refined_count,
                          void* workspace, size_t workspace_bytes, float coarse_margin, void* coarse, size_t coarse_bytes,
                          int32_t* visited_count, fr_stream_t stream);
+int fr_pnet23_coarse_tiles_f16(const float* x1, const void* x1s, int B, int H1, int W1, const float* w2, const float* b2, const float* s2,
+                               const float* w3, const float* b3, const float* s3, const float* hw, const float* hb,
+                               float* head, int all_heads, float refine_logit_thr, float refine_band_hi, int32_t* refined_count,
+                               void* workspace, size_t workspace_bytes, float coarse_margin, void* coarse, size_t coarse_bytes,
+                               int tile_rows, int32_t* visited_count, fr_stream_t stream);
 int fr_maxpool_f32(const float* x, float* y, int B, int H, int W, int C, int k, int stride,
                    fr_stream_t stream);
 int fr_pnet_candidates(const float* head, int nframes, int hc, int wc, float scale, float thr, int cap,
@@ -291,6 +296,10 @@
                                const float* w3, const float* b3, const float* s3, const float* hw, const float* hb, int all_heads,
                                float refine_logit_thr, float refine_band_hi, float coarse_margin, void* const* coarse,
                                int32_t* visited_count, fr_stream_t stream);
+int fr_pnet_pyramid_p23_coarse_tiles(const fr_pnet_level* levels, int nlevels, int nframes, const float* w2, const float* b2,
+                                     const float* s2, const float* w3, const float* b3, const float* s3, const float* hw,
+                                     const float* hb, int all_heads, float refine_logit_thr, float refine_band_hi, float coarse_margin,
+                                     void* const* coarse, const int32_t* tile_rows, int32_t* visited_count, fr_stream_t stream);
 
 int fr_letterbox_u8(const fr_frame_ref* refs, int nframes, uint8_t* canvas, int dh, int dw, fr_stream_t stream);
 int fr_detections_unscale(float* boxes, float* kps, const int32_t* counts, const float* det_scale, int nframes, int cap,
```

Result: no change. 26950 (-0.3%).
